# martinsbruveris/tensorflow-image-models

Measured on AMD Instinct MI355X. Metric: images/sec (fwd, bf16), higher is better.
Workload: dtype bf16; 1 GPU; resnet50 @224 fwd; per_gpu_batch=256, global_batch=256, parallelism=dp1, exchange=none, ranks=1, launcher=in-process, launch=hipGraph replay, 2 parallel branches of 128 images, branches=2

## Files before the change

### include/tfimm_hip.h

```cpp
#ifndef TFIMM_HIP_H
#define TFIMM_HIP_H

#include <stddef.h>
#include <stdint.h>

#ifdef __cplusplus
extern "C" {
#endif

#define TFIMM_HIP_ABI_VERSION 4

#if defined(__GNUC__)
#define TFIMM_API __attribute__((visibility("default")))
#else
#define TFIMM_API
#endif

#define TFIMM_EINVAL (-1)
#define TFIMM_EUNSUP (-2)

enum {
  TFIMM_ACT_NONE = 0,
  TFIMM_ACT_RELU = 1,
  TFIMM_ACT_GELU = 2,
// ... 152 lines not shown
  int64_t in_bytes;
  int64_t w_floats;
  int32_t B, c_in, H, W, c_out;
  int32_t pad_t, pad_b, pad_l, pad_r;
  int32_t taps_cap;
  int32_t lds_bytes;
} tfimm_resize_batch_aa_desc;

typedef struct tfimm_resize_batch_sizes {
  int64_t in_bytes;
  int64_t tab_elems;
  int64_t w_floats;
  int64_t n_tiles;
  int32_t max_taps;
  int32_t lds_floats;
  int32_t bad_image;
  int32_t reserved;
} tfimm_resize_batch_sizes;

TFIMM_API int tfimm_hip_resize_batch_tables(int B, const int32_t* src_hw, const int32_t* geometry, int H, int W, int c_in,
                                            const int32_t* pad, int method, int antialias, tfimm_resize_batch_sizes* sizes,
                                            tfimm_resize_batch_rec* recs, int32_t* tab_a, int32_t* tab_b, float* w);
TFIMM_API int tfimm_hip_preprocess_resize_batch(const tfimm_resize_batch_desc* d, void* stream);
TFIMM_API int tfimm_hip_preprocess_resize_batch_aa(const tfimm_resize_batch_aa_desc* d, void* stream);

typedef struct tfimm_resize_region_rec {
  int64_t in_offset;
  int64_t row_pitch;
  int32_t Hs, Ws;
  int32_t y_tab, x_tab;
  int32_t y_w, x_w;
  int32_t y_taps, x_taps;
  int32_t tile_rows;
  int32_t cols_max;
  int32_t tile0, n_tiles;
} tfimm_resize_region_rec;

typedef struct tfimm_resize_region_desc {
  const void* in;
  const tfimm_resize_region_rec* recs;
  void* out;
  const int32_t* idx;
  const float* w;
  const float* mean_host;
  const float* std_host;
  int64_t in_bytes;
  int32_t B, c_in, H, W, c_out;
  int32_t pad_t, pad_b, pad_l, pad_r;
  int32_t taps;
} tfimm_resize_region_desc;

typedef struct tfimm_resize_region_aa_desc {
  const void* in;
  const tfimm_resize_region_rec* recs;
  void* out;
  const int32_t* start;
  const int32_t* count;
  const float* w;
  const float* mean_host;
  const float* std_host;
  int64_t in_bytes;
  int64_t w_floats;
  int32_t B, c_in, H, W, c_out;
  int32_t pad_t, pad_b, pad_l, pad_r;
  int32_t taps_cap;
  int32_t lds_bytes;
} tfimm_resize_region_aa_desc;

TFIMM_API int tfimm_hip_resize_region_tables(int F, const int32_t* frame_hw, int N, const int32_t* boxes,
                                             const int32_t* box_frame, const int32_t* geometry, int H, int W, int c_in,
                                             const int32_t* pad, int method, int antialias, tfimm_resize_batch_sizes* sizes,
                                             tfimm_resize_region_rec* recs, int32_t* tab_a, int32_t* tab_b, float* w);
TFIMM_API int tfimm_hip_preprocess_regions(const tfimm_resize_region_desc* d, void* stream);
TFIMM_API int tfimm_hip_preprocess_regions_aa(const tfimm_resize_region_aa_desc* d, void* stream);

TFIMM_API int tfimm_hip_layernorm(const void* x, void* y, const float* gamma, const float* beta,
                        int64_t rows, int d, int64_t x_stride, int64_t y_stride, float eps,
                        void* stream);

typedef struct tfimm_attn_desc {
  const void* qkv;
  void* out;
  const float* rel_bias;
  int32_t batch;
  int32_t n_tokens;
  int32_t heads, hd;
  float scale;
  int32_t window, shift, res_h, res_w;
  const float* bias_log2;
} tfimm_attn_desc;

TFIMM_API int tfimm_hip_attention(const tfimm_attn_desc* d, void* stream);

typedef struct tfimm_tha_desc {
  const void* qkv;
  void* out;
  const float* proj_l_w;
  const float* proj_l_b;
  const float* proj_w_w;
  const float* proj_w_b;
  int32_t batch, n_tokens, heads, hd;
  float scale;
  const float* proj_dev;
} tfimm_tha_desc;

TFIMM_API int tfimm_hip_talking_heads_attention(const tfimm_tha_desc* d, void* stream);

TFIMM_API int tfimm_hip_class_attention(const void* q, const void* kv, void* out, int B, int n_tokens, int heads,
                              int hd, int ldq, int ldkv, int ldo, void* stream);

TFIMM_API int tfimm_hip_copy_rows(const void* src, void* dst, int B, int src_rows, int dst_rows, int dst_row0,
                        int d, void* stream);

TFIMM_API int tfimm_hip_maxpool(const void* x, void* y, int B, int H, int W, int C, int k, int stride,
                      int pad, int OH, int OW, void* stream);

TFIMM_API int tfimm_hip_mean_rows(const void* x, void* y, int B, int R, int C, int out_f32, void* stream);

TFIMM_API int tfimm_hip_bcast_rows(const void* src, void* dst, int B, int n_rows, int d,
                         int dst_rows_per_image, void* stream);

TFIMM_API int tfimm_hip_dwconv(const void* x, const float* w, const float* bias, void* y, void* sum_out,
                     int B, int H, int W, int C, int k, int stride, int pad_t, int pad_l,
                     int OH, int OW, int act, void* stream);

TFIMM_API int tfimm_hip_se_gate(const void* sums, int sums_fixed, float inv_count, const float* w1, const float* b1,
                      const float* w2, const float* b2, float* gate, int B, int C, int rd,
                      int act, int gate_act, void* stream);

TFIMM_API int tfimm_hip_scale_channels(const void* x, const float* gate, const void* residual, void* y,
                             int B, int R, int C, int act_after, void* stream);

TFIMM_API int tfimm_hip_patch_merge_ln(const void* x, void* y, const float* gamma, const float* beta,
                             int B, int H, int W, int C, float eps, void* stream);

typedef struct tfimm_chain_desc {
  const void* x;
  const void* w1;
  const float* b1;
  const void* w2;
  const float* b2;
  const void* residual;
  void* out;
  int32_t B, H, W, Cin, KH, KW, stride, pad_t, pad_l, OH, OW;
  int32_t C1, N2;
  int32_t ldw1, ldw2, ldr, ldc;
  int32_t act1, act2;
  const void* ds_x;
  const void* ds_w;
  int32_t ds_cin;
} tfimm_chain_desc;

TFIMM_API int tfimm_hip_conv_chain(const tfimm_chain_desc* d, void* stream);

typedef struct tfimm_expand_dw_desc {
  const void* x;
  const void* w1;
  const float* b1;
  const float* wdw;
  const float* b2;
  void* y;
  void* sum_out;
  int32_t B, H, W, Cin, C, Cpad, k, stride, pad_t, pad_l, OH, OW;
  int32_t act1, act2;
  int32_t stem;
  int32_t img_h, img_w;
} tfimm_expand_dw_desc;

TFIMM_API int tfimm_hip_expand_dwconv(const tfimm_expand_dw_desc* d, void* stream);

TFIMM_API int tfimm_hip_attention_probs(const void* qkv, void* probs, int B, int n_tokens, int heads, int hd,
                              float scale, void* stream);

TFIMM_API int tfimm_hip_group_norm(const void* x, const float* gamma, const float* beta, const void* residual, void* y,
                         void* stats_ws, int B, int rows, int C, int groups, float eps, int act,
                         int act_after_res, void* stream);

TFIMM_API int tfimm_hip_blur_pool(const void* x, void* y, int B, int H, int W, int C, int stride, void* stream);

TFIMM_API int tfimm_hip_avg_pool(const void* x, void* y, int B, int H, int W, int C, int k, int stride, void* stream);

TFIMM_API int tfimm_hip_eca_gate(const float* sums, float inv_count, const float* w, float* gate, int B, int C, int k,
                       int gate_act, void* stream);

TFIMM_API int tfimm_hip_grouped_conv3x3(const void* x, const void* wfrag, const float* bias, void* y, int B, int H, int W,
                              int C, int stride, int act, void* stream);

TFIMM_API int tfimm_hip_memset_async(void* dst, int value, size_t bytes, void* stream);

TFIMM_API int tfimm_hip_bias_act(const void* x, const float* bias, void* y, int64_t rows, int C, int act,
                       void* stream);

typedef struct tfimm_mlp_desc {
  const void* x;
  const void* w1;
  const float* b1;
  const void* w2;
  const float* b2;
  const void* residual;
  void* out;
  int64_t M;
  int32_t C, hidden, act;
  float eps;
} tfimm_mlp_desc;
TFIMM_API int tfimm_hip_mlp_fused(const tfimm_mlp_desc* d, void* stream);


TFIMM_API int tfimm_hip_quantize_mx(const void* x, int64_t rows, int C, int64_t x_stride, const float* gamma,
                                    const float* beta, float eps, void* q, void* q_scale, int ldq, void* stream);

typedef struct tfimm_gemm_mx_desc {
  const void* a;
  const void* a_scale;
  const void* w;
  const void* w_scale;
  const float* bias;
  const void* residual;
  void* out;
  void* out_scale;
  int32_t M, N, K;
  int32_t lda, ldw, ldr, ldc;
  int32_t out_fmt;
  int32_t act, act_after_res;
} tfimm_gemm_mx_desc;
TFIMM_API int tfimm_hip_gemm_mx(const tfimm_gemm_mx_desc* d, void* stream);


#define TFIMM_TOPK_MAX_K 64
#define TFIMM_TOPK_MAX_N 32768
TFIMM_API int tfimm_hip_topk(const float* logits, int64_t ld, int B, int N, int k, float* values, int32_t* indices,
                             float* probs, void* stream);

#define TFIMM_SCORE_MAX_N TFIMM_TOPK_MAX_N
#define TFIMM_SCORE_MAX_CONFUSION_N 4096
#define TFIMM_SCORE_IGNORE (-1)
#define TFIMM_SCORE_SCORED 0
#define TFIMM_SCORE_IGNORED 1
#define TFIMM_SCORE_INVALID 2
#define TFIMM_SCORE_LOSS_EXCLUDED 3
#define TFIMM_SCORE_LOSS_Q 4
#define TFIMM_SCORE_RANK_HIST 5
#define TFIMM_SCORE_RANK_BINS 65
#define TFIMM_SCORE_STATE_WORDS 70
TFIMM_API int tfimm_hip_score(const float* logits, int64_t ld, int B, int N, const int32_t* labels, float* loss, int32_t* rank,
                              int32_t* pred, float* prob, int64_t* state, int64_t* per_class, uint32_t* confusion, void* stream);


TFIMM_API int tfimm_hip_softmax_grad(const float* logits, int64_t ld, int B, int N, const int32_t* labels, void* grad, int64_t ldg,
                                     float* loss, int32_t* pred, void* stream);

#define TFIMM_HEAD_SGD 0
#define TFIMM_HEAD_ADAM 1
#define TFIMM_HEAD_MAX_D 8192
#define TFIMM_HEAD_MAX_C 32768
#define TFIMM_HEAD_MAX_B 65535
typedef struct tfimm_head_update_desc {
  const void* f;
  const void* g;
  const int32_t* labels;
  float* w;
  void* w16;
  float* s1;
  float* s2;
  float* bias;
  float* bias_s1;
  float* bias_s2;
  float* grad_out;
  float* bias_grad_out;
  int32_t B, D, C;
  int32_t ldf, ldg, ldw, ldw16;
  int32_t opt;
  float lr, mom_or_one_minus_b1, one_minus_b2, eps, wd2;
} tfimm_head_update_desc;
TFIMM_API int tfimm_hip_head_update(const tfimm_head_update_desc* d, void* stream);

#define TFIMM_DISTILL_MAX_E 4096
TFIMM_API int tfimm_hip_distill_grad(const float* s, int64_t ld_s, const float* t, int64_t ld_t, int B, int E, const int32_t* valid,
                                     int normalize, void* grad, int64_t ldg, float* loss, float* cosine, void* stream);


TFIMM_API int tfimm_hip_l2_normalize(const float* x, int64_t ld_x, int B, int E, float* y, int64_t ld_y, void* stream);

#define TFIMM_EMBED_MIN_E 16
#define TFIMM_EMBED_MAX_E 2048
#define TFIMM_EMBED_MAX_K 64
#define TFIMM_EMBED_MAX_B 2097120
TFIMM_API int64_t tfimm_hip_embed_search_workspace(int B, int N, int E, int k, int chunk);
TFIMM_API int tfimm_hip_embed_search(const float* q, int64_t ld_q, int B, const void* g, int64_t ld_g, int N, int E, int k, int chunk,
                                     float* scores, int32_t* indices, void* workspace, int64_t workspace_bytes, void* stream);

#define TFIMM_EMBED_WIDE_MAX_K 256
TFIMM_API int tfimm_hip_embed_search_wide_max_k(int E);
TFIMM_API int64_t tfimm_hip_embed_search_wide_workspace(int B, int N, int E, int k, int chunk);
TFIMM_API int tfimm_hip_embed_search_wide(const float* q, int64_t ld_q, int B, const void* g, int64_t ld_g, int N, int E, int k,
                                          int chunk, float* scores, int32_t* indices, void* workspace, int64_t workspace_bytes,
                                          void* stream);

#define TFIMM_EMBED_COARSE_MAX_CANDIDATES 256
TFIMM_API int tfimm_hip_embed_quantize_rows(const void* g, int64_t ld_g, int N, int E, void* codes, int64_t ld_c, int8_t* exps,
                                            void* stream);
TFIMM_API int tfimm_hip_embed_search_coarse_max_candidates(int E);
TFIMM_API int64_t tfimm_hip_embed_search_coarse_workspace(int B, int N, int E, int k, int candidates, int chunk);
TFIMM_API int tfimm_hip_embed_search_coarse(const float* q, int64_t ld_q, int B, const void* g, int64_t ld_g, const void* codes,
                                            int64_t ld_c, const int8_t* exps, int N, int E, int k, int candidates, int chunk,
                                            float* scores, int32_t* indices, void* workspace, int64_t workspace_bytes, void* stream);

// ... 95 lines not shown
```

### tensorflow-image-models_amd/csrc/gemm_chain.hip

```cpp
#include "gemm_chain_kernel.h"

#include <algorithm>
#include <cstdlib>

using namespace tfimm_gemm;

namespace {
int chain_num_cu() {
  static int n = 0;
  if (n == 0) {
    int dev = 0;
    hipDeviceProp_t prop;
    if (hipGetDevice(&dev) == hipSuccess && hipGetDeviceProperties(&prop, dev) == hipSuccess) n = prop.multiProcessorCount;
    if (n <= 0) n = 256;
  }
  return n;
}
}

int tfimm_launch_conv_strip_chain(const tfimm_chain_desc& d, int64_t M, int num_cu, hipStream_t stream);

extern "C" int tfimm_hip_conv_chain(const tfimm_chain_desc* dp, void* stream) {
  if (!dp) TFIMM_FAIL(TFIMM_EINVAL, "conv_chain: null descriptor");
  const tfimm_chain_desc& d = *dp;
  if (!d.x || !d.w1 || !d.b1 || !d.w2 || !d.b2 || !d.out) TFIMM_FAIL(TFIMM_EINVAL, "conv_chain: null pointer");
  if (d.B <= 0 || d.H <= 0 || d.W <= 0 || d.Cin <= 0 || d.KH <= 0 || d.KW <= 0 || d.stride <= 0 || d.OH <= 0 || d.OW <= 0 ||
      d.C1 <= 0 || d.N2 <= 0)
    TFIMM_FAIL(TFIMM_EINVAL, "conv_chain: bad shape");
  if (d.C1 == 128) {
    if (d.Cin != 128 || d.KH != 3 || d.KW != 3 || d.stride != 1 || d.pad_t != 1 || d.pad_l != 1 || d.OH != d.H || d.OW != d.W)
      TFIMM_FAIL(TFIMM_EUNSUP, "conv_chain: C1 = 128 is built for a 3x3 / stride 1 / pad 1 convolution over 128 -> 128 channels");
    if (d.W > 31) TFIMM_FAIL(TFIMM_EUNSUP, "conv_chain: C1 = 128 needs W <= 31 (W = %d): the strip of a 128-pixel tile must fit 192 LDS rows", d.W);
    if (d.N2 != 256 && d.N2 != 512) TFIMM_FAIL(TFIMM_EUNSUP, "conv_chain: N2 = %d (built: 256, 512)", d.N2);
    if (d.ds_x || d.ds_w) TFIMM_FAIL(TFIMM_EUNSUP, "conv_chain: the shortcut-convolution flavour exists for C1 = 64 only");
    if (d.ldw1 != 1152) TFIMM_FAIL(TFIMM_EINVAL, "conv_chain: ldw1 = %d, expected KH*KW*Cin = 1152", d.ldw1);
    if (d.ldw2 < 128 || (d.ldw2 & 7)) TFIMM_FAIL(TFIMM_EINVAL, "conv_chain: ldw2 = %d", d.ldw2);
    if (d.ldc < d.N2 || (d.ldc & 7) || (d.residual && (d.ldr < d.N2 || (d.ldr & 7))))
      TFIMM_FAIL(TFIMM_EINVAL, "conv_chain: output / residual rows must be 16-byte aligned (ldc = %d, ldr = %d)", d.ldc, d.ldr);
    if (((uintptr_t)d.x | (uintptr_t)d.w1 | (uintptr_t)d.w2 | (uintptr_t)d.out | (uintptr_t)d.residual | (uintptr_t)d.b1 | (uintptr_t)d.b2) & 15)
      TFIMM_FAIL(TFIMM_EINVAL, "conv_chain: pointers must be 16-byte aligned");
    const int64_t M = (int64_t)d.B * d.OH * d.OW;
    const int64_t big = std::max<int64_t>(M * 256, ((M - 1) * std::max(d.ldc, d.ldr) + d.N2) * 2);
    static const int64_t lim128 = getenv("TFIMM_CHAIN_LIMIT") ? std::min<int64_t>(atoll(getenv("TFIMM_CHAIN_LIMIT")), 0x7fffff00LL) : 0x7fffff00LL;
    if (big > lim128) {
      const int64_t per_img = (int64_t)d.OH * d.OW * std::max<int64_t>(256, (int64_t)std::max(d.ldc, d.ldr) * 2);
      const int64_t chunk = lim128 / per_img;
      if (chunk < 1 || d.B <= 1) TFIMM_FAIL(TFIMM_EUNSUP, "conv_chain: one image exceeds the 2 GiB a buffer descriptor addresses");
      for (int64_t b0 = 0; b0 < d.B; b0 += chunk) {
        tfimm_chain_desc c = d;
        c.B = (int32_t)std::min<int64_t>(chunk, d.B - b0);
        c.x = (const char*)d.x + b0 * d.H * d.W * 256;
        c.out = (char*)d.out + b0 * d.OH * d.OW * d.ldc * 2;
        if (d.residual) c.residual = (const char*)d.residual + b0 * d.OH * d.OW * d.ldr * 2;
        const int rc = tfimm_hip_conv_chain(&c, stream);
        if (rc != 0) return rc;
      }
      return 0;
    }
    return tfimm_launch_conv_strip_chain(d, M, chain_num_cu(), (hipStream_t)stream);
  }
  if (d.C1 != 64 || d.Cin != 64 || d.KH != 3 || d.KW != 3 || d.stride != 1 || d.pad_t != 1 || d.pad_l != 1 || d.OH != d.H ||
      d.OW != d.W)
    TFIMM_FAIL(TFIMM_EUNSUP, "conv_chain: built for a 3x3 / stride 1 / pad 1 convolution over 64 -> 64 channels");
  if (d.W > 63) TFIMM_FAIL(TFIMM_EUNSUP, "conv_chain: W = %d > 63 (the input strip of a 128-pixel tile must fit 256 LDS rows)", d.W);
  if (d.N2 != 256 && d.N2 != 512) TFIMM_FAIL(TFIMM_EUNSUP, "conv_chain: N2 = %d (built: 256, 512)", d.N2);
  const int64_t K1 = 576;
  if (d.ldw1 != K1) TFIMM_FAIL(TFIMM_EINVAL, "conv_chain: ldw1 = %d, expected KH*KW*Cin = %lld", d.ldw1, (long long)K1);
  if (d.ldw2 < d.C1 || (d.ldw2 & 7)) TFIMM_FAIL(TFIMM_EINVAL, "conv_chain: ldw2 = %d", d.ldw2);
  if (d.ldc < d.N2 || (d.ldc & 7) || (d.residual && (d.ldr < d.N2 || (d.ldr & 7))))
    TFIMM_FAIL(TFIMM_EINVAL, "conv_chain: output / residual rows must be 16-byte aligned (ldc = %d, ldr = %d)", d.ldc, d.ldr);
  if (((uintptr_t)d.x | (uintptr_t)d.w1 | (uintptr_t)d.w2 | (uintptr_t)d.out | (uintptr_t)d.residual | (uintptr_t)d.b1 |
       (uintptr_t)d.b2) & 15)
    TFIMM_FAIL(TFIMM_EINVAL, "conv_chain: pointers must be 16-byte aligned");
  const int64_t M = (int64_t)d.B * d.OH * d.OW;
  const int64_t x_bytes = (int64_t)d.B * d.H * d.W * d.Cin * 2;
  const int64_t w1_bytes = (int64_t)d.C1 * d.ldw1 * 2, w2_bytes = (int64_t)d.N2 * d.ldw2 * 2;
  const int64_t out_bytes = ((M - 1) * d.ldc + d.N2) * 2;
  const int64_t res_bytes = d.residual ? ((M - 1) * d.ldr + d.N2) * 2 : 0;
  const bool ds = d.ds_x != nullptr;
  if (ds != (d.ds_w != nullptr)) TFIMM_FAIL(TFIMM_EINVAL, "conv_chain: ds_x and ds_w go together");
  if (ds && (d.residual || d.ds_cin != 64 || (((uintptr_t)d.ds_x | (uintptr_t)d.ds_w) & 15)))
    TFIMM_FAIL(TFIMM_EUNSUP, "conv_chain: the shortcut convolution is built for a 64-channel block input and no other residual");
  if (ds && !(d.act1 == TFIMM_ACT_RELU && d.act2 == TFIMM_ACT_RELU))
    TFIMM_FAIL(TFIMM_EUNSUP, "conv_chain: the shortcut-convolution flavour is built with relu activations");
  if (w1_bytes > 0x7fffff00LL || w2_bytes > 0x7fffff00LL)
    TFIMM_FAIL(TFIMM_EUNSUP, "conv_chain: a weight tensor exceeds the 2 GiB a buffer descriptor addresses");
  static const int64_t limit = getenv("TFIMM_CHAIN_LIMIT") ? std::min<int64_t>(atoll(getenv("TFIMM_CHAIN_LIMIT")), 0x7fffff00LL) : 0x7fffff00LL;
  if (M > limit || x_bytes > limit || out_bytes > limit || res_bytes > limit) {
    const int64_t per_img = std::max<int64_t>(std::max<int64_t>((int64_t)d.H * d.W * d.Cin * 2, (int64_t)d.OH * d.OW * d.ldc * 2),
                                              d.residual ? (int64_t)d.OH * d.OW * d.ldr * 2 : 0);
    const int64_t chunk = limit / per_img;
    if (chunk < 1 || d.B <= 1) TFIMM_FAIL(TFIMM_EUNSUP, "conv_chain: one image exceeds the 2 GiB a buffer descriptor addresses");
    for (int64_t b0 = 0; b0 < d.B; b0 += chunk) {
      tfimm_chain_desc c = d;
      c.B = (int32_t)std::min<int64_t>(chunk, d.B - b0);
      c.x = (const char*)d.x + b0 * d.H * d.W * d.Cin * 2;
      c.out = (char*)d.out + b0 * d.OH * d.OW * d.ldc * 2;
      if (d.residual) c.residual = (const char*)d.residual + b0 * d.OH * d.OW * d.ldr * 2;
      if (d.ds_x) c.ds_x = (const char*)d.ds_x + b0 * d.OH * d.OW * d.ds_cin * 2;
      const int rc = tfimm_hip_conv_chain(&c, stream);
      if (rc != 0) return rc;
    }
    return 0;
  }

  ChainArgs a;
  a.x = (const bf16_t*)d.x; a.w1 = (const bf16_t*)d.w1; a.b1 = d.b1;
  a.w2 = (const bf16_t*)d.w2; a.b2 = d.b2; a.residual = (const bf16_t*)d.residual; a.out = (bf16_t*)d.out;
  a.ds_x = (const bf16_t*)d.ds_x; a.ds_w = (const uint4*)d.ds_w; a.ds_bytes = ds ? (unsigned)(M * 128) : 0u;
  a.M = (int)M; a.N2 = d.N2;
  a.B = d.B; a.H = d.H; a.W = d.W;
  a.ldw1 = d.ldw1; a.ldw2 = d.ldw2; a.ldr = d.ldr; a.ldc = d.ldc;
  a.act1 = d.act1; a.act2 = d.act2;
  a.x_bytes = (unsigned)x_bytes; a.w1_bytes = (unsigned)w1_bytes; a.w2_bytes = (unsigned)w2_bytes;
  a.out_bytes = (unsigned)out_bytes; a.res_bytes = (unsigned)res_bytes;
  a.n_tiles = (int)cdiv64(M, 128);
  {
    static const int dbg = getenv("TFIMM_CHAIN_DBG") ? atoi(getenv("TFIMM_CHAIN_DBG")) : 0;
    a.dbg = dbg;
  }

  const int vi = d.N2 == 512;
  const int ri = (d.act1 == TFIMM_ACT_RELU && d.act2 == TFIMM_ACT_RELU) ? 1 : 0;
  const gemm_chain_fn fn = ds ? (vi ? gemm_chain_kernel<8, TFIMM_ACT_RELU, true> : gemm_chain_kernel<4, TFIMM_ACT_RELU, true>)
                           : ri ? (vi ? gemm_chain_kernel<8, TFIMM_ACT_RELU> : gemm_chain_kernel<4, TFIMM_ACT_RELU>)
                                : (vi ? gemm_chain_kernel<8> : gemm_chain_kernel<4>);
  const int lds = ChainGeom::LDS_BYTES;
  static tfimm_once_t ready[2][3];
  const int fi = ds ? 2 : ri;
  if (ready[vi][fi].need()) {
    TFIMM_HIP_CHECK(hipFuncSetAttribute((const void*)fn, hipFuncAttributeMaxDynamicSharedMemorySize, lds));
    ready[vi][fi].mark();
  }
  int64_t grid = ((int64_t)chain_num_cu() * 2 + 7) / 8 * 8;
  const int64_t need = ((int64_t)a.n_tiles + 7) / 8 * 8;
  if (grid > need) grid = need;
  TFIMM_LAUNCH(fn, dim3((unsigned)grid), dim3(256), (size_t)lds, (hipStream_t)stream, a);
  return 0;
}
```

### tensorflow-image-models_amd/csrc/gemm_chain_kernel.h

```cpp
#pragma once
#include "gemm_stream_kernel.h"

namespace tfimm_gemm {

struct ChainArgs {
  const bf16_t* x;
  const bf16_t* w1;
  const float* b1;
  const bf16_t* w2;
  const float* b2;
  const bf16_t* residual;
  const bf16_t* ds_x;
  const uint4* ds_w;
  bf16_t* out;
  int M, N2;
  int B, H, W;
  int ldw1, ldw2, ldr, ldc;
  int act1, act2;
  unsigned x_bytes, w1_bytes, w2_bytes, out_bytes, res_bytes, ds_bytes;
  int n_tiles;
  int dbg;
};

typedef void (*gemm_chain_fn)(const ChainArgs);

struct ChainGeom {
  static constexpr int BM = 128, NW = 4, C1 = 64, BN2 = 64;
  static constexpr int STRIP_ROWS = 256;
  static constexpr int STRIP_BYTES = STRIP_ROWS * 128;
  static constexpr int STAGE = 64 * 128;
#ifndef TFIMM_CHAIN_NST
#define TFIMM_CHAIN_NST 2
#endif
#ifndef TFIMM_CHAIN_WTN
#define TFIMM_CHAIN_WTN 64
#endif
  static constexpr int NST = TFIMM_CHAIN_NST;
  static constexpr int WTN = TFIMM_CHAIN_WTN;
  static constexpr int EPI_WAVE = 32 * WTN * 4;
  static constexpr int LDS_BYTES = STRIP_BYTES + NST * STAGE + NW * EPI_WAVE;
  static_assert(LDS_BYTES <= 80 * 1024, "two workgroups must fit one CU's 160 KiB of LDS");
};

template <int N>
__device__ __forceinline__ void chain_wait_vm() {
  asm volatile("s_waitcnt vmcnt(%0)" ::"n"(N) : "memory");
}

template <int I>
struct ChainIdx {
  static constexpr int value = I;
};

template <int NS2, int ACT = -1, bool DS = false>
__global__ void __launch_bounds__(256, 2) gemm_chain_kernel(const ChainArgs p) {
  using G = ChainGeom;
  constexpr int BM = G::BM, NW = G::NW, STAGE = G::STAGE, BN2 = G::BN2, NST = G::NST;
  constexpr int TN1 = 2;
  constexpr int STRIP_INSTR = G::STRIP_ROWS / 8 / NW;
  constexpr int B1_INSTR = 64 / 8 / NW;
  constexpr int B2_INSTR = BN2 / 8 / NW;
  constexpr int KS2 = 4;
  constexpr int TN2 = BN2 / 32;
  constexpr int NK1 = 9;
  typedef __attribute__((ext_vector_type(4))) unsigned int u32x4;

  extern __shared__ __attribute__((aligned(16))) char smem[];
  char* const sRing = smem + G::STRIP_BYTES;
  float* const sEpi = reinterpret_cast<float*>(smem + G::STRIP_BYTES + NST * STAGE);

  const int tid = threadIdx.x;
  const int lane = tid & 63;
  const int wave = __builtin_amdgcn_readfirstlane(tid >> 6);
  const int frow = lane & 31, fhi = lane >> 5;

  int t_first, t_hi, t_step;
  {
    const int nb = gridDim.x, bid = blockIdx.x;
    const int xcd = bid & 7, j = bid >> 3;
    const int q = p.n_tiles >> 3, r = p.n_tiles & 7;
    const int t_lo = xcd * q + (xcd < r ? xcd : r);
    t_hi = t_lo + q + (xcd < r ? 1 : 0);
    t_step = nb >> 3;
    t_first = t_lo + j;
  }
  if (t_first >= t_hi) return;

  const __amdgpu_buffer_rsrc_t rsrc_x = make_rsrc(p.x, p.x_bytes);
  const __amdgpu_buffer_rsrc_t rsrc_w1 = make_rsrc(p.w1, p.w1_bytes);
  const __amdgpu_buffer_rsrc_t rsrc_w2 = make_rsrc(p.w2, p.w2_bytes);
  const __amdgpu_buffer_rsrc_t rsrc_o = make_rsrc(p.out, p.out_bytes);
  const __amdgpu_buffer_rsrc_t rsrc_r = DS ? make_rsrc(p.ds_x, p.ds_bytes) : make_rsrc(p.residual, p.res_bytes);

  static_assert(NS2 >= 2, "the counted waits below are derived for at least two GEMM-2 steps");
  constexpr int LOOK = NST - 1;
  const int lrow = lane >> 3, lpc = lane & 7;

  unsigned b1_off[B1_INSTR], b2_off[B2_INSTR];
  int strip_chunk[STRIP_INSTR];
#pragma unroll
  for (int j = 0; j < B1_INSTR; ++j) {
    const int r = (wave * B1_INSTR + j) * 8 + lrow;
    b1_off[j] = (unsigned)(((size_t)r * p.ldw1 + (lpc ^ ((r >> 1) & 7)) * 8) * 2);
  }
#pragma unroll
  for (int j = 0; j < B2_INSTR; ++j) {
    const int r = (wave * B2_INSTR + j) * 8 + lrow;
    b2_off[j] = (unsigned)(((size_t)r * p.ldw2 + (lpc ^ ((r >> 1) & 7)) * 8) * 2);
  }
#pragma unroll
  for (int j = 0; j < STRIP_INSTR; ++j) {
    const int r = (wave * STRIP_INSTR + j) * 8 + lrow;
    strip_chunk[j] = (lpc ^ ((r >> 1) & 7)) * 16;
  }
  const int halo = p.W + 1;
  const int n_pix = p.B * p.H * p.W;
  auto issue_strip = [&](int tile, bool valid) __attribute__((always_inline)) {
    const int s0 = tile * BM - halo;
#pragma unroll
    for (int j = 0; j < STRIP_INSTR; ++j) {
      const int r = (wave * STRIP_INSTR + j) * 8 + lrow;
      const int s = s0 + r;
      const bool ok = valid && s >= 0 && s < n_pix;
      const unsigned off = ok ? (unsigned)s * 128u + (unsigned)strip_chunk[j] : kOobOffset;
      __builtin_amdgcn_raw_ptr_buffer_load_lds(rsrc_x, (lds_ptr_t)(smem + (wave * STRIP_INSTR + j) * 1024), 16, (int)off, 0, 0, 0);
    }
  };
  int iss_stage = 0;
  auto issue_step = [&](auto sc, int tile) __attribute__((always_inline)) {
    constexpr int S = decltype(sc)::value;
    constexpr int SL = S >= NK1 + NS2 ? S - NK1 - NS2 : S;
    const bool valid = S >= NK1 + NS2 ? (tile + t_step < t_hi) : true;
    char* const sa = sRing + iss_stage * STAGE;
    if constexpr (SL < NK1) {
#pragma unroll
      for (int j = 0; j < B1_INSTR; ++j) {
        const unsigned off = valid ? b1_off[j] : kOobOffset;
        __builtin_amdgcn_raw_ptr_buffer_load_lds(rsrc_w1, (lds_ptr_t)(sa + (wave * B1_INSTR + j) * 1024), 16, (int)off, SL * 128, 0, 0);
      }
    } else {
      const int soff = (int)((size_t)(SL - NK1) * BN2 * p.ldw2 * 2);
#pragma unroll
      for (int j = 0; j < B2_INSTR; ++j)
        __builtin_amdgcn_raw_ptr_buffer_load_lds(rsrc_w2, (lds_ptr_t)(sa + (wave * B2_INSTR + j) * 1024), 16, (int)b2_off[j], soff, 0, 0);
    }
    iss_stage = iss_stage == NST - 1 ? 0 : iss_stage + 1;
  };

  constexpr int WTN = G::WTN, LPR = WTN / 8, RPI = 64 / LPR, ITS = 32 / RPI;
  constexpr int PASSES = BN2 / WTN;
  constexpr int BPP = WTN / 32;
  constexpr int STORES = PASSES * ITS;
  constexpr int DS_X = DS ? 4 : 0;
  constexpr int DS_W = DS ? 8 : 0;
  constexpr int EPI_LOADS = (DS ? 0 : PASSES * ITS) + PASSES * 2;
  auto epi_slot = [](int row, int slot) -> int { return WTN == 64 ? (slot ^ (row & 15)) : (slot ^ ((row >> 1) & 7)); };
  const ActParams act1p = make_act(ACT >= 0 ? ACT : p.act1), act2p = make_act(ACT >= 0 ? ACT : p.act2);
  const int e_row = lane / LPR, e_c8 = lane % LPR;
  const bool has_res = !DS && p.residual != nullptr;
  float* const sEw = sEpi + wave * (G::EPI_WAVE / 4);

  struct Ops {
    static constexpr int all(int r) {
      if (DS && r == NK1 - 2) return B1_INSTR + TN1 * 4;
      if (r < NK1 - 1) return B1_INSTR;
      if (r == NK1 - 1) return EPI_LOADS + DS_X + B1_INSTR;
      const int u = r - NK1;
      return (u < NS2 - 1 ? EPI_LOADS : 0) + DS_W + B2_INSTR + (u == 0 ? STRIP_INSTR : 0) + STORES;
    }
    static constexpr int behind_dma(int r) {
      if (r < NK1) return 0;
      return (r - NK1 == 0 ? STRIP_INSTR : 0) + STORES;
    }
    static constexpr int wait_for(int r) {
      constexpr int T = NK1 + NS2;
      int n = behind_dma((r + T - LOOK) % T);
      for (int i = 1; i < LOOK; ++i) n += all((r + T - i) % T);
      return n;
    }
  };
  static_assert(B1_INSTR == B2_INSTR, "every weight step is two pieces per wave");
  static_assert(Ops::wait_for(NK1 + NS2 - 1) < 64, "vmcnt is a 6-bit counter");

  f32x4 bias1[TN1][4];
  auto load_bias1 = [&]() __attribute__((always_inline)) {
#pragma unroll
    for (int j = 0; j < TN1; ++j)
#pragma unroll
      for (int q = 0; q < 4; ++q) {
        const float4 b4 = *reinterpret_cast<const float4*>(p.b1 + j * 32 + q * 8 + fhi * 4);
        bias1[j][q] = f32x4{b4.x, b4.y, b4.z, b4.w};
      }
  };
  if constexpr (!DS) {
    load_bias1();
    asm volatile("s_waitcnt vmcnt(0)" : "+v"(bias1[0][0]), "+v"(bias1[0][3]), "+v"(bias1[TN1 - 1][0]), "+v"(bias1[TN1 - 1][3])::"memory");
  }

  if (TFIMM_PROBE(p.dbg) & 8) {
    const int n = ((blockIdx.x >> 3) & 7) * (TFIMM_PROBE(p.dbg) >> 8);
    for (int i = 0; i < n; ++i) asm volatile("s_sleep 8");
  }
  issue_strip(t_first, true);
  issue_step(ChainIdx<0>{}, t_first);
  if constexpr (LOOK > 1) issue_step(ChainIdx<1>{}, t_first);
  if constexpr (LOOK > 2) issue_step(ChainIdx<2>{}, t_first);
  static_assert(LOOK >= 1 && LOOK <= 3, "prologue written for up to three steps of lookahead");
  int cur = 0;
  bool first = true;
  auto rotate = [&]() __attribute__((always_inline)) { cur = cur == NST - 1 ? 0 : cur + 1; };

  for (int tile = t_first; tile < t_hi; tile += t_step) {
    const int m0 = tile * BM;

    unsigned vmask;
    {
      const int m = m0 + wave * 32 + frow;
      const int hw = p.H * p.W;
      const int rem = m % hw;
      const int oy = rem / p.W, ox = rem - oy * p.W;
      const unsigned vy = (oy > 0 ? 1u : 0u) | 2u | (oy + 1 < p.H ? 4u : 0u);
      const unsigned vx = (ox > 0 ? 1u : 0u) | 2u | (ox + 1 < p.W ? 4u : 0u);
      vmask = 0;
#pragma unroll
      for (int ky = 0; ky < 3; ++ky)
        if ((vy >> ky) & 1) vmask |= vx << (3 * ky);
      if (m >= p.M) vmask = 0;
    }

    f32x16 acc1[TN1];
#pragma unroll
    for (int j = 0; j < TN1; ++j)
#pragma unroll
      for (int e = 0; e < 16; ++e) acc1[j][e] = 0.f;
    uint4 rres[2][PASSES][ITS];
    u32x4 dsx[4];
    float4 braw[2][PASSES][2];
    const int e_m = m0 + wave * 32 + e_row;
    const int em = e_m < p.M ? e_m : p.M;
    const unsigned ldc2 = (unsigned)p.ldc * 2u, ldr2 = (unsigned)p.ldr * 2u;
    auto load_epi = [&](auto uc) __attribute__((always_inline)) {
      constexpr int u = decltype(uc)::value;
      const unsigned res_off0 = (unsigned)(((size_t)em * p.ldr + u * BN2 + e_c8 * 8) * 2);
#pragma unroll
      for (int g = 0; g < PASSES; ++g) {
        if constexpr (!DS) {
#pragma unroll
        for (int it = 0; it < ITS; ++it) {
          const unsigned off = res_off0 + (unsigned)(it * RPI) * ldr2 + (unsigned)(g * WTN * 2);
          rres[u & 1][g][it] = __builtin_bit_cast(uint4, __builtin_amdgcn_raw_buffer_load_b128(rsrc_r, (int)((TFIMM_PROBE(p.dbg) & 4) ? kOobOffset : off), 0, 0));
        }
        }
        braw[u & 1][g][0] = *reinterpret_cast<const float4*>(p.b2 + u * BN2 + g * WTN + e_c8 * 8);
        braw[u & 1][g][1] = *reinterpret_cast<const float4*>(p.b2 + u * BN2 + g * WTN + e_c8 * 8 + 4);
      }
    };
    auto tap_step = [&](auto kc) __attribute__((always_inline)) {
      constexpr int k = decltype(kc)::value;
      if constexpr (k < LOOK) { if (first) chain_wait_vm<(LOOK - 1) * B1_INSTR>(); else chain_wait_vm<Ops::wait_for(k)>(); }
      else chain_wait_vm<Ops::wait_for(k)>();
      tfimm_lds_reuse_barrier();
      if constexpr (DS && k == NK1 - 2) { load_bias1(); __builtin_amdgcn_sched_barrier(0); }
      if constexpr (k == NK1 - 1) {
        load_epi(ChainIdx<0>{});
        if constexpr (DS) {
          const unsigned xo = (unsigned)(m0 + wave * 32 + frow) * 128u + (unsigned)fhi * 16u;
#pragma unroll
          for (int t = 0; t < 4; ++t) dsx[t] = __builtin_amdgcn_raw_buffer_load_b128(rsrc_r, (int)(xo + t * 32), 0, 0);
        }
        __builtin_amdgcn_sched_barrier(0);
      }
      issue_step(ChainIdx<k + LOOK>{}, tile);
      if constexpr (k == NK1 - 1) __builtin_amdgcn_sched_barrier(0);
      constexpr int ky = k / 3, kx = k % 3;
      const bool ok = (vmask >> k) & 1;
      const uint4* sB = reinterpret_cast<const uint4*>(sRing + cur * STAGE);
      const int arow = wave * 32 + frow + ky * p.W + kx;
      u32x4 ua[4];
      {
        unsigned ra[4];
#pragma unroll
        for (int ks = 0; ks < 4; ++ks) ra[ks] = (unsigned)(size_t)(lds_ptr_t)(smem + lds_slot(arow, ks * 2 + fhi) * 16);
        asm volatile("ds_read_b128 %0, %4\n\tds_read_b128 %1, %5\n\tds_read_b128 %2, %6\n\tds_read_b128 %3, %7\n\t"
                     "s_waitcnt lgkmcnt(0)"
                     : "=&v"(ua[0]), "=&v"(ua[1]), "=&v"(ua[2]), "=&v"(ua[3])
                     : "v"(ra[0]), "v"(ra[1]), "v"(ra[2]), "v"(ra[3]) : "memory");
      }
#pragma unroll
      for (int ks = 0; ks < 4; ++ks) {
        const uint4 um = sel4(ok, __builtin_bit_cast(uint4, ua[ks]));
        const bf16x8 fa = __builtin_bit_cast(bf16x8, um);
        bf16x8 fb[TN1];
#pragma unroll
        for (int j = 0; j < TN1; ++j) fb[j] = __builtin_bit_cast(bf16x8, sB[lds_slot(j * 32 + frow, ks * 2 + fhi)]);
#pragma unroll
        for (int j = 0; j < TN1; ++j)
          if (!(TFIMM_PROBE(p.dbg) & 2)) acc1[j] = __builtin_amdgcn_mfma_f32_32x32x16_bf16(fb[j], fa, acc1[j], 0, 0, 0);
      }
      rotate();
    };
    tap_step(ChainIdx<0>{}); tap_step(ChainIdx<1>{}); tap_step(ChainIdx<2>{}); tap_step(ChainIdx<3>{}); tap_step(ChainIdx<4>{});
    tap_step(ChainIdx<5>{}); tap_step(ChainIdx<6>{}); tap_step(ChainIdx<7>{}); tap_step(ChainIdx<8>{});
    bf16x8 bmid[KS2];
#pragma unroll
    for (int j = 0; j < TN1; ++j)
#pragma unroll
      for (int q2 = 0; q2 < 2; ++q2) {
        tfimm_f32x2 v[4];
#pragma unroll
        for (int h2 = 0; h2 < 2; ++h2) {
          const int q = q2 * 2 + h2;
          const f32x4 b4 = bias1[j][q];
          v[h2 * 2 + 0] = tfimm_f32x2{acc1[j][q * 4 + 0] + b4[0], acc1[j][q * 4 + 1] + b4[1]};
          v[h2 * 2 + 1] = tfimm_f32x2{acc1[j][q * 4 + 2] + b4[2], acc1[j][q * 4 + 3] + b4[3]};
        }
        act8p(v, act1p);
        bmid[j * 2 + q2] = __builtin_bit_cast(bf16x8, pack8p(v));
      }

    auto slice_step = [&](auto uc) __attribute__((always_inline)) {
      constexpr int u = decltype(uc)::value;
      constexpr int n0 = u * BN2;
      const unsigned out_off0 = (unsigned)(((size_t)em * p.ldc + n0 + e_c8 * 8) * 2);
      chain_wait_vm<Ops::wait_for(NK1 + u)>();
      tfimm_lds_reuse_barrier();
      if constexpr (u + 1 < NS2) load_epi(ChainIdx<u + 1>{});
      u32x4 wds[TN2][4];
      if constexpr (DS) {
#pragma unroll
        for (int j = 0; j < TN2; ++j)
#pragma unroll
          for (int t = 0; t < 4; ++t) wds[j][t] = __builtin_bit_cast(u32x4, p.ds_w[(size_t)((u * TN2 + j) * 4 + t) * 64 + lane]);
      }
      __builtin_amdgcn_sched_barrier(0);
      issue_step(ChainIdx<NK1 + u + LOOK>{}, tile);
      if constexpr (u == 0) issue_strip(tile + t_step, tile + t_step < t_hi);
      __builtin_amdgcn_sched_barrier(0);

      f32x16 acc[TN2];
#pragma unroll
      for (int j = 0; j < TN2; ++j)
#pragma unroll
        for (int e = 0; e < 16; ++e) acc[j][e] = 0.f;
      {
        const uint4* sW = reinterpret_cast<const uint4*>(sRing + cur * STAGE);
#pragma unroll
        for (int t = 0; t < KS2; ++t) {
          bf16x8 fw[TN2];
#pragma unroll
          for (int j = 0; j < TN2; ++j) fw[j] = __builtin_bit_cast(bf16x8, sW[lds_slot(j * 32 + frow, t * 2 + fhi)]);
#pragma unroll
          for (int j = 0; j < TN2; ++j) acc[j] = __builtin_amdgcn_mfma_f32_32x32x16_bf16(fw[j], bmid[t], acc[j], 0, 0, 0);
        }
      }
      if constexpr (DS) {
#pragma unroll
        for (int t = 0; t < 4; ++t)
#pragma unroll
          for (int j = 0; j < TN2; ++j)
            acc[j] = __builtin_amdgcn_mfma_f32_32x32x16_bf16(__builtin_bit_cast(bf16x8, wds[j][t]), __builtin_bit_cast(bf16x8, dsx[t]),
                                                             acc[j], 0, 0, 0);
      }
      rotate();

      const bool skip_epi = (TFIMM_PROBE(p.dbg) & 1) != 0;
#pragma unroll
      for (int g = 0; g < PASSES; ++g) {
        asm volatile("s_nop 15\n\ts_nop 3" : "+v"(acc[g * BPP]), "+v"(acc[g * BPP + BPP - 1]));
#pragma unroll
        for (int j = 0; j < BPP; ++j)
#pragma unroll
          for (int q = 0; q < 4; ++q) {
            const int slot = j * 8 + q * 2 + fhi;
            const f32x16& a16 = acc[g * BPP + j];
            const f32x4 v = {a16[q * 4 + 0], a16[q * 4 + 1], a16[q * 4 + 2], a16[q * 4 + 3]};
            const unsigned addr = (unsigned)(size_t)(lds_ptr_t)(&sEw[frow * WTN + epi_slot(frow, slot) * 4]);
            asm volatile("ds_write_b128 %0, %1" ::"v"(addr), "v"(v) : "memory");
          }
        const float4 bq0 = braw[u & 1][g][0], bq1 = braw[u & 1][g][1];
        const tfimm_f32x2 bias2[4] = {{bq0.x, bq0.y}, {bq0.z, bq0.w}, {bq1.x, bq1.y}, {bq1.z, bq1.w}};
#pragma unroll
        for (int ip = 0; ip < ITS; ip += 2) {
        f32x4 st[4];
        {
          unsigned ra[4];
#pragma unroll
          for (int w = 0; w < 2; ++w) {
            const int pr = (ip + w) * RPI + e_row;
            ra[2 * w] = (unsigned)(size_t)(lds_ptr_t)(&sEw[pr * WTN + epi_slot(pr, 2 * e_c8) * 4]);
            ra[2 * w + 1] = (unsigned)(size_t)(lds_ptr_t)(&sEw[pr * WTN + epi_slot(pr, 2 * e_c8 + 1) * 4]);
          }
          asm volatile("ds_read_b128 %0, %4\n\tds_read_b128 %1, %5\n\tds_read_b128 %2, %6\n\tds_read_b128 %3, %7\n\t"
                       "s_waitcnt lgkmcnt(0)"
                       : "=&v"(st[0]), "=&v"(st[1]), "=&v"(st[2]), "=&v"(st[3])
                       : "v"(ra[0]), "v"(ra[1]), "v"(ra[2]), "v"(ra[3]) : "memory");
        }
#pragma unroll
        for (int w = 0; w < 2; ++w) {
          const int it = ip + w;
          const f32x4 lo = st[2 * w], hi = st[2 * w + 1];
          tfimm_f32x2 v[4] = {{lo[0], lo[1]}, {lo[2], lo[3]}, {hi[0], hi[1]}, {hi[2], hi[3]}};
#pragma unroll
          for (int e = 0; e < 4; ++e) v[e] += bias2[e];
          if (has_res) {
            asm volatile("");
            tfimm_f32x2 r2[4];
            unpack8p(rres[u & 1][g][it], r2);
#pragma unroll
            for (int e = 0; e < 4; ++e) v[e] += r2[e];
          }
          act8p(v, act2p);
          const unsigned off = out_off0 + (unsigned)(it * RPI) * ldc2 + (unsigned)(g * WTN * 2);
          __builtin_amdgcn_raw_buffer_store_b128(__builtin_bit_cast(u32x4, pack8p(v)), rsrc_o,
                                                 (int)(skip_epi ? kOobOffset : off), 0, 0);
        }
        }
      }
    };
    slice_step(ChainIdx<0>{});
    slice_step(ChainIdx<1>{});
    if constexpr (NS2 > 2) slice_step(ChainIdx<2>{});
    if constexpr (NS2 > 3) slice_step(ChainIdx<3>{});
    if constexpr (NS2 > 4) { slice_step(ChainIdx<4>{}); slice_step(ChainIdx<5>{}); slice_step(ChainIdx<6>{}); slice_step(ChainIdx<7>{}); }
    static_assert(NS2 == 2 || NS2 == 3 || NS2 == 4 || NS2 == 8, "instantiate the slice steps of this NS2");
    first = false;
  }
  asm volatile("s_waitcnt vmcnt(0)" ::: "memory");
}

}
```

### tensorflow-image-models_amd/csrc/plan.hip

```cpp
#include "common.h"

#include <cstring>
#include <map>
#include <string>
#include <utility>
#include <vector>

namespace {

constexpr uint32_t kMagic = 0x4c504654u;
constexpr uint32_t kVersion = 1;
enum ArgKind : uint32_t { A_INT = 0, A_FLOAT = 1, A_NULL = 2, A_SLAB = 3, A_CONST = 4, A_HOST = 5, A_INPUT = 6, A_STRUCT = 7 };

struct Reader {
  const uint8_t* p;
  const uint8_t* end;
  bool ok = true;
  template <typename T> T get() {
    T v{};
    if (p + sizeof(T) > end) { ok = false; return v; }
    memcpy(&v, p, sizeof(T));
    p += sizeof(T);
    return v;
  }
  std::string str() {
    const uint32_t n = get<uint32_t>();
    if (!ok || p + n > end) { ok = false; return std::string(); }
    std::string s(reinterpret_cast<const char*>(p), n);
    p += n;
    return s;
  }
};

struct ArgSpec { uint32_t kind, aux; uint64_t value; };
struct Arg { int64_t i; double f; void* p; };
struct Reloc { uint32_t field_offset, kind, aux; uint64_t value; };
struct StructSpec { std::vector<uint8_t> bytes; std::vector<Reloc> relocs; };
struct Output { std::string name; uint32_t slab; uint64_t offset; uint64_t rows_per_image, cols; uint32_t dtype; };

typedef int (*adapter_fn)(const Arg*, void*);
struct Call { adapter_fn fn; std::string name; std::vector<ArgSpec> spec; std::vector<Arg> args; bool is_memset = false; };

template <typename T> T as(const Arg& a) {
  if constexpr (std::is_pointer<T>::value) return reinterpret_cast<T>(a.p);
  else if constexpr (std::is_floating_point<T>::value) return static_cast<T>(a.f);
  else return static_cast<T>(a.i);
}
template <typename... P, size_t... I>
int invoke_impl(int (*fn)(P..., void*), const Arg* a, void* stream, std::index_sequence<I...>) {
  return fn(as<P>(a[I])..., stream);
}
template <typename R, typename... P> constexpr size_t arity(R (*)(P...)) { return sizeof...(P) - 1; }

#define TFIMM_ADAPTER(NAME, ...)                                                                          \
  {#NAME, {[](const Arg* a, void* s) -> int {                                                             \
             return invoke_impl<__VA_ARGS__>(NAME, a, s, std::make_index_sequence<arity(NAME)>{});       \
           }, arity(NAME), 0}}
#define TFIMM_ADAPTER_DESC(NAME, DESC)                                                                    \
  {#NAME, {[](const Arg* a, void* s) -> int {                                                             \
             return invoke_impl<const DESC*>(NAME, a, s, std::make_index_sequence<arity(NAME)>{});       \
           }, arity(NAME), sizeof(DESC)}}

struct Entry { adapter_fn fn; size_t nargs; size_t desc_bytes; };

const std::map<std::string, Entry>& table() {
  using vp = const void*;
  using mp = void*;
  using fp = const float*;
  static const std::map<std::string, Entry> t = {
      TFIMM_ADAPTER_DESC(tfimm_hip_gemm, tfimm_gemm_desc),
      TFIMM_ADAPTER_DESC(tfimm_hip_conv_chain, tfimm_chain_desc),
      TFIMM_ADAPTER_DESC(tfimm_hip_mlp_fused, tfimm_mlp_desc),
      TFIMM_ADAPTER_DESC(tfimm_hip_gemm_mx, tfimm_gemm_mx_desc),
      TFIMM_ADAPTER_DESC(tfimm_hip_expand_dwconv, tfimm_expand_dw_desc),
      TFIMM_ADAPTER_DESC(tfimm_hip_stem_conv_pool, tfimm_stem_desc),
      TFIMM_ADAPTER_DESC(tfimm_hip_attention, tfimm_attn_desc),
      TFIMM_ADAPTER_DESC(tfimm_hip_talking_heads_attention, tfimm_tha_desc),
      TFIMM_ADAPTER(tfimm_hip_cast_input, vp, int, mp, int64_t, int, int),
      TFIMM_ADAPTER(tfimm_hip_cast_input_pad, vp, int, mp, int, int, int, int, int, int, int, int),
      TFIMM_ADAPTER(tfimm_hip_row_stats, vp, float*, int64_t, int, int64_t, float),
      TFIMM_ADAPTER(tfimm_hip_quantize_mx, vp, int64_t, int, int64_t, fp, fp, float, mp, mp, int),
      TFIMM_ADAPTER(tfimm_hip_layernorm, vp, mp, fp, fp, int64_t, int, int64_t, int64_t, float),
      TFIMM_ADAPTER(tfimm_hip_class_attention, vp, vp, mp, int, int, int, int, int, int, int),
      TFIMM_ADAPTER(tfimm_hip_copy_rows, vp, mp, int, int, int, int, int),
      TFIMM_ADAPTER(tfimm_hip_maxpool, vp, mp, int, int, int, int, int, int, int, int, int),
      TFIMM_ADAPTER(tfimm_hip_mean_rows, vp, mp, int, int, int, int),
      TFIMM_ADAPTER(tfimm_hip_bcast_rows, vp, mp, int, int, int, int),
      TFIMM_ADAPTER(tfimm_hip_dwconv, vp, fp, fp, mp, mp, int, int, int, int, int, int, int, int, int, int, int),
      TFIMM_ADAPTER(tfimm_hip_se_gate, vp, int, float, fp, fp, fp, fp, float*, int, int, int, int, int),
      TFIMM_ADAPTER(tfimm_hip_scale_channels, vp, fp, vp, mp, int, int, int, int),
      TFIMM_ADAPTER(tfimm_hip_patch_merge_ln, vp, mp, fp, fp, int, int, int, int, float),
      TFIMM_ADAPTER(tfimm_hip_attention_probs, vp, mp, int, int, int, int, float),
      TFIMM_ADAPTER(tfimm_hip_group_norm, vp, fp, fp, vp, mp, mp, int, int, int, int, float, int, int),
      TFIMM_ADAPTER(tfimm_hip_blur_pool, vp, mp, int, int, int, int, int),
      TFIMM_ADAPTER(tfimm_hip_avg_pool, vp, mp, int, int, int, int, int, int),
      TFIMM_ADAPTER(tfimm_hip_eca_gate, fp, float, fp, float*, int, int, int, int),
      TFIMM_ADAPTER(tfimm_hip_grouped_conv3x3, vp, vp, fp, mp, int, int, int, int, int, int),
      TFIMM_ADAPTER(tfimm_hip_bias_act, vp, fp, mp, int64_t, int, int),
      TFIMM_ADAPTER(tfimm_hip_topk, fp, int64_t, int, int, int, float*, int32_t*, float*),
  };
  return t;
}

struct Plan {
  uint32_t batch = 0;
  std::vector<uint64_t> slab_bytes, slab_off;
  std::vector<uint64_t> const_bytes, const_off, const_src;
  std::vector<std::vector<uint8_t>> host_consts;
  std::vector<StructSpec> structs;
  std::vector<Call> calls;
  std::vector<Output> outputs;
  int32_t input_call = -1;
  int32_t stem_call = -1, stem_struct = -1;
  int32_t img_h = 0, img_w = 0, img_c = 0, stem_pad_t = 0, stem_pad_l = 0;
  uint64_t workspace_bytes = 0;
  char* ws = nullptr;
};

uint64_t align256(uint64_t v) { return (v + 255) / 256 * 256; }

int parse(const void* blob, size_t bytes, Plan& pl) {
  Reader r{static_cast<const uint8_t*>(blob), static_cast<const uint8_t*>(blob) + bytes};
  if (r.get<uint32_t>() != kMagic) TFIMM_FAIL(TFIMM_EINVAL, "plan: not a plan blob");
  if (r.get<uint32_t>() != kVersion) TFIMM_FAIL(TFIMM_EINVAL, "plan: blob version mismatch");
  if ((int)r.get<uint32_t>() != tfimm_hip_abi_version()) TFIMM_FAIL(TFIMM_EINVAL, "plan: exported for another ABI version");
  pl.batch = r.get<uint32_t>();
  pl.img_h = r.get<int32_t>(); pl.img_w = r.get<int32_t>(); pl.img_c = r.get<int32_t>();
  constexpr uint64_t kMaxBuf = 1ull << 40;
  uint64_t off = 0;
  for (uint32_t i = 0, n = r.get<uint32_t>(); i < n && r.ok; ++i) {
    pl.slab_bytes.push_back(r.get<uint64_t>());
    pl.slab_off.push_back(off);
    if (pl.slab_bytes.back() > kMaxBuf || off > kMaxBuf) TFIMM_FAIL(TFIMM_EINVAL, "plan: slab %u of %llu bytes", i, (unsigned long long)pl.slab_bytes.back());
    off += align256(pl.slab_bytes.back());
  }
  for (uint32_t i = 0, n = r.get<uint32_t>(); i < n && r.ok; ++i) {
    pl.const_bytes.push_back(r.get<uint64_t>());
    pl.const_src.push_back(r.get<uint64_t>());
    pl.const_off.push_back(off);
    if (pl.const_bytes.back() > bytes || pl.const_src.back() > bytes - pl.const_bytes.back())
      TFIMM_FAIL(TFIMM_EINVAL, "plan: constant outside the blob");
    if (pl.const_bytes.back() > kMaxBuf || off > kMaxBuf) TFIMM_FAIL(TFIMM_EINVAL, "plan: workspace too large");
    off += align256(pl.const_bytes.back());
  }
  pl.workspace_bytes = off;
  for (uint32_t i = 0, n = r.get<uint32_t>(); i < n && r.ok; ++i) {
    const uint64_t nb = r.get<uint64_t>(), src = r.get<uint64_t>();
    if (nb > bytes || src > bytes - nb) TFIMM_FAIL(TFIMM_EINVAL, "plan: host constant outside the blob");
    pl.host_consts.emplace_back(static_cast<const uint8_t*>(blob) + src, static_cast<const uint8_t*>(blob) + src + nb);
  }
  for (uint32_t i = 0, n = r.get<uint32_t>(); i < n && r.ok; ++i) {
    StructSpec s;
    const uint32_t nb = r.get<uint32_t>(), nr = r.get<uint32_t>();
    if (!r.ok || nb > (size_t)(r.end - r.p)) TFIMM_FAIL(TFIMM_EINVAL, "plan: truncated struct");
    s.bytes.assign(r.p, r.p + nb);
    r.p += nb;
    for (uint32_t k = 0; k < nr && r.ok; ++k) {
      Reloc rl;
      rl.field_offset = r.get<uint32_t>(); rl.kind = r.get<uint32_t>(); rl.aux = r.get<uint32_t>(); rl.value = r.get<uint64_t>();
      if (nb < sizeof(void*) || rl.field_offset > nb - sizeof(void*)) TFIMM_FAIL(TFIMM_EINVAL, "plan: relocation outside its struct");
      s.relocs.push_back(rl);
    }
    pl.structs.push_back(std::move(s));
  }
  for (uint32_t i = 0, n = r.get<uint32_t>(); i < n && r.ok; ++i) {
    Call c;
    c.name = r.str();
    const uint32_t na = r.get<uint32_t>();
    for (uint32_t k = 0; k < na && r.ok; ++k) {
      ArgSpec a;
      a.kind = r.get<uint32_t>(); a.aux = r.get<uint32_t>(); a.value = r.get<uint64_t>();
      c.spec.push_back(a);
    }
    if (c.name == "memset") {
      c.is_memset = true;
      c.fn = nullptr;
      if (na != 2) TFIMM_FAIL(TFIMM_EINVAL, "plan: memset takes (pointer, bytes)");
    } else {
      const auto it = table().find(c.name);
      if (it == table().end()) TFIMM_FAIL(TFIMM_EUNSUP, "plan: no executor entry for %s", c.name.c_str());
      if (it->second.nargs != na) TFIMM_FAIL(TFIMM_EINVAL, "plan: %s takes %zu arguments, blob has %u", c.name.c_str(), it->second.nargs, na);
      c.fn = it->second.fn;
    }
    pl.calls.push_back(std::move(c));
  }
  pl.input_call = r.get<int32_t>();
  pl.stem_call = r.get<int32_t>(); pl.stem_struct = r.get<int32_t>();
  pl.stem_pad_t = r.get<int32_t>(); pl.stem_pad_l = r.get<int32_t>();
  for (uint32_t i = 0, n = r.get<uint32_t>(); i < n && r.ok; ++i) {
    Output o;
    o.name = r.str();
    o.slab = r.get<uint32_t>(); o.offset = r.get<uint64_t>(); o.rows_per_image = r.get<uint64_t>(); o.cols = r.get<uint64_t>();
    o.dtype = r.get<uint32_t>();
    pl.outputs.push_back(o);
  }
  if (!r.ok) TFIMM_FAIL(TFIMM_EINVAL, "plan: truncated blob");
  if (pl.input_call < 0 || pl.input_call >= (int)pl.calls.size()) TFIMM_FAIL(TFIMM_EINVAL, "plan: no input call");
  if (pl.calls[pl.input_call].spec.size() < 2) TFIMM_FAIL(TFIMM_EINVAL, "plan: the input call takes (pointer, dtype, ...)");
  if (pl.stem_call >= 0) {
    if (pl.stem_call >= (int)pl.calls.size() || pl.stem_struct < 0 || pl.stem_struct >= (int)pl.structs.size() ||
        pl.structs[pl.stem_struct].bytes.size() < sizeof(tfimm_stem_desc))
      TFIMM_FAIL(TFIMM_EINVAL, "plan: bad stem reference");
  }
  for (const auto& o : pl.outputs) {
    if (o.slab >= pl.slab_off.size()) TFIMM_FAIL(TFIMM_EINVAL, "plan: output '%s' outside its slab", o.name.c_str());
    if (o.dtype > 2) TFIMM_FAIL(TFIMM_EINVAL, "plan: output '%s' has dtype code %u (0 bf16, 1 fp32, 2 int32)", o.name.c_str(), o.dtype);
    const uint64_t cap = pl.slab_bytes[o.slab], esz = o.dtype == 0 ? 2 : 4;
    bool ok = o.offset < cap && o.cols > 0 && o.rows_per_image > 0 && pl.batch > 0 && o.cols <= kMaxBuf && o.rows_per_image <= kMaxBuf / pl.batch;
    if (ok) {
      const uint64_t rows = o.rows_per_image * (uint64_t)pl.batch;
      ok = o.cols <= kMaxBuf / rows && rows * o.cols <= (cap - o.offset) / esz;
    }
    if (!ok) TFIMM_FAIL(TFIMM_EINVAL, "plan: output '%s' outside its slab", o.name.c_str());
  }
  for (const auto& c : pl.calls) {
    if (c.is_memset) continue;
    const auto& e = table().find(c.name)->second;
    for (size_t k = 0; k < c.spec.size(); ++k)
      if (c.spec[k].kind == A_STRUCT) {
        if (c.spec[k].aux >= pl.structs.size()) TFIMM_FAIL(TFIMM_EINVAL, "plan: bad struct reference");
        if (e.desc_bytes && pl.structs[c.spec[k].aux].bytes.size() < e.desc_bytes)
          TFIMM_FAIL(TFIMM_EINVAL, "plan: %s descriptor has %zu bytes, the entry point reads %zu", c.name.c_str(),
                     pl.structs[c.spec[k].aux].bytes.size(), e.desc_bytes);
      }
// ... 132 lines not shown
```

### tensorflow-image-models_amd/tfimm/engine/ffi.py

```python
import ctypes as C
import os

import torch

_HERE = os.path.dirname(os.path.abspath(__file__))
LIB_PATH = os.environ.get("TFIMM_HIP_LIB") or os.path.join(_HERE, "libtfimm_hip.so")

ACT = {
    "": 0, "linear": 0, "none": 0, None: 0,
    "relu": 1, "gelu": 2, "swish": 3, "sigmoid": 4, "relu6": 5, "tanh": 6,
}
A_DENSE, A_CONV, A_CONV_C4 = 0, 1, 2


class GemmDesc(C.Structure):
    _fields_ = [
        ("a", C.c_void_p), ("wt", C.c_void_p), ("bias", C.c_void_p), ("residual", C.c_void_p),
        ("out", C.c_void_p), ("a_scale", C.c_void_p),
        ("M", C.c_int32), ("N", C.c_int32), ("K", C.c_int32),
        ("lda", C.c_int32), ("ldw", C.c_int32), ("ldr", C.c_int32), ("ldc", C.c_int32),
        ("out_f32", C.c_int32), ("act", C.c_int32), ("act_after_res", C.c_int32),
        ("res_mod", C.c_int32),
        ("remap_in", C.c_int32), ("remap_out", C.c_int32), ("remap_off", C.c_int32),
        ("mode", C.c_int32),
        ("B", C.c_int32), ("H", C.c_int32), ("W", C.c_int32), ("Cin", C.c_int32),
        ("KH", C.c_int32), ("KW", C.c_int32), ("stride", C.c_int32),
        ("pad_t", C.c_int32), ("pad_l", C.c_int32), ("OH", C.c_int32), ("OW", C.c_int32),
        ("rows_per_image", C.c_int32), ("tile_hint", C.c_int32), ("stride_w", C.c_int32),
        ("pix_pitch", C.c_int32),
        ("ln_stats", C.c_void_p), ("ln_c1", C.c_void_p),
        ("a2", C.c_void_p), ("K2", C.c_int32), ("lda2", C.c_int32),
        ("a2_stride", C.c_int32), ("a2_H", C.c_int32), ("a2_W", C.c_int32), ("a2_OH", C.c_int32), ("a2_OW", C.c_int32),
        ("a2_window", C.c_int32),
    ]


class AttnDesc(C.Structure):
    _fields_ = [
        ("qkv", C.c_void_p), ("out", C.c_void_p), ("rel_bias", C.c_void_p),
        ("batch", C.c_int32), ("n_tokens", C.c_int32), ("heads", C.c_int32), ("hd", C.c_int32),
        ("scale", C.c_float),
        ("window", C.c_int32), ("shift", C.c_int32), ("res_h", C.c_int32), ("res_w", C.c_int32),
        ("bias_log2", C.c_void_p),
    ]


class ThaDesc(C.Structure):
    _fields_ = [
        ("qkv", C.c_void_p), ("out", C.c_void_p),
        ("proj_l_w", C.c_void_p), ("proj_l_b", C.c_void_p), ("proj_w_w", C.c_void_p), ("proj_w_b", C.c_void_p),
        ("batch", C.c_int32), ("n_tokens", C.c_int32), ("heads", C.c_int32), ("hd", C.c_int32),
        ("scale", C.c_float), ("proj_dev", C.c_void_p),
    ]


class StemDesc(C.Structure):
    _fields_ = [
        ("x", C.c_void_p), ("wt", C.c_void_p), ("bias", C.c_void_p), ("out", C.c_void_p),
        ("batch", C.c_int32), ("Hp", C.c_int32), ("Wp2", C.c_int32), ("OH", C.c_int32), ("OW", C.c_int32),
        ("ldw", C.c_int32),
        ("in_dtype", C.c_int32), ("H", C.c_int32), ("W", C.c_int32), ("pad_t", C.c_int32), ("pad_l", C.c_int32),
    ]


class ChainDesc(C.Structure):
    _fields_ = [
        ("x", C.c_void_p), ("w1", C.c_void_p), ("b1", C.c_void_p), ("w2", C.c_void_p), ("b2", C.c_void_p),
        ("residual", C.c_void_p), ("out", C.c_void_p),
        ("B", C.c_int32), ("H", C.c_int32), ("W", C.c_int32), ("Cin", C.c_int32), ("KH", C.c_int32), ("KW", C.c_int32),
        ("stride", C.c_int32), ("pad_t", C.c_int32), ("pad_l", C.c_int32), ("OH", C.c_int32), ("OW", C.c_int32),
        ("C1", C.c_int32), ("N2", C.c_int32),
        ("ldw1", C.c_int32), ("ldw2", C.c_int32), ("ldr", C.c_int32), ("ldc", C.c_int32),
        ("act1", C.c_int32), ("act2", C.c_int32),
        ("ds_x", C.c_void_p), ("ds_w", C.c_void_p), ("ds_cin", C.c_int32),
    ]


class ExpandDwDesc(C.Structure):
    _fields_ = [
        ("x", C.c_void_p), ("w1", C.c_void_p), ("b1", C.c_void_p), ("wdw", C.c_void_p), ("b2", C.c_void_p),
        ("y", C.c_void_p), ("sum_out", C.c_void_p),
        ("B", C.c_int32), ("H", C.c_int32), ("W", C.c_int32), ("Cin", C.c_int32), ("C", C.c_int32), ("Cpad", C.c_int32),
        ("k", C.c_int32), ("stride", C.c_int32), ("pad_t", C.c_int32), ("pad_l", C.c_int32), ("OH", C.c_int32),
        ("OW", C.c_int32), ("act1", C.c_int32), ("act2", C.c_int32),
        ("stem", C.c_int32), ("img_h", C.c_int32), ("img_w", C.c_int32),
    ]


class MlpDesc(C.Structure):
    _fields_ = [("x", C.c_void_p), ("w1", C.c_void_p), ("b1", C.c_void_p), ("w2", C.c_void_p),
                ("b2", C.c_void_p), ("residual", C.c_void_p), ("out", C.c_void_p), ("M", C.c_int64),
                ("C", C.c_int32), ("hidden", C.c_int32), ("act", C.c_int32), ("eps", C.c_float)]


class GemmMxDesc(C.Structure):
    _fields_ = [("a", C.c_void_p), ("a_scale", C.c_void_p), ("w", C.c_void_p), ("w_scale", C.c_void_p),
                ("bias", C.c_void_p), ("residual", C.c_void_p), ("out", C.c_void_p), ("out_scale", C.c_void_p),
                ("M", C.c_int32), ("N", C.c_int32), ("K", C.c_int32),
                ("lda", C.c_int32), ("ldw", C.c_int32), ("ldr", C.c_int32), ("ldc", C.c_int32),
                ("out_fmt", C.c_int32), ("act", C.c_int32), ("act_after_res", C.c_int32)]


class LoraDesc(C.Structure):
    _fields_ = [("x", C.c_void_p), ("a", C.c_void_p), ("b", C.c_void_p), ("residual", C.c_void_p), ("out", C.c_void_p),
                ("M", C.c_int64), ("K", C.c_int32), ("N", C.c_int32), ("Rp", C.c_int32),
                ("lda", C.c_int32), ("lda_a", C.c_int32), ("ldr", C.c_int32), ("ldc", C.c_int32)]


class HeadUpdateDesc(C.Structure):
    _fields_ = [("f", C.c_void_p), ("g", C.c_void_p), ("labels", C.c_void_p),
                ("w", C.c_void_p), ("w16", C.c_void_p), ("s1", C.c_void_p), ("s2", C.c_void_p),
                ("bias", C.c_void_p), ("bias_s1", C.c_void_p), ("bias_s2", C.c_void_p),
                ("grad_out", C.c_void_p), ("bias_grad_out", C.c_void_p),
                ("B", C.c_int32), ("D", C.c_int32), ("C", C.c_int32),
                ("ldf", C.c_int32), ("ldg", C.c_int32), ("ldw", C.c_int32), ("ldw16", C.c_int32),
                ("opt", C.c_int32),
                ("lr", C.c_float), ("mom_or_one_minus_b1", C.c_float), ("one_minus_b2", C.c_float), ("eps", C.c_float),
                ("wd2", C.c_float)]


class ResizeDesc(C.Structure):
    _fields_ = [("in_", C.c_void_p), ("out", C.c_void_p),
                ("y_idx", C.c_void_p), ("y_w", C.c_void_p), ("x_idx", C.c_void_p), ("x_w", C.c_void_p),
                ("mean_host", C.POINTER(C.c_float)), ("std_host", C.POINTER(C.c_float)),
                ("B", C.c_int32), ("Hs", C.c_int32), ("Ws", C.c_int32), ("c_in", C.c_int32),
                ("H", C.c_int32), ("W", C.c_int32), ("c_out", C.c_int32),
                ("pad_t", C.c_int32), ("pad_b", C.c_int32), ("pad_l", C.c_int32), ("pad_r", C.c_int32),
                ("taps", C.c_int32)]


class ResizeAADesc(C.Structure):
    _fields_ = [("in_", C.c_void_p), ("out", C.c_void_p),
                ("y_start", C.c_void_p), ("y_count", C.c_void_p), ("y_w", C.c_void_p),
                ("x_start", C.c_void_p), ("x_count", C.c_void_p), ("x_w", C.c_void_p),
                ("mean_host", C.POINTER(C.c_float)), ("std_host", C.POINTER(C.c_float)),
                ("B", C.c_int32), ("Hs", C.c_int32), ("Ws", C.c_int32), ("c_in", C.c_int32),
                ("H", C.c_int32), ("W", C.c_int32), ("c_out", C.c_int32),
                ("pad_t", C.c_int32), ("pad_b", C.c_int32), ("pad_l", C.c_int32), ("pad_r", C.c_int32),
                ("y_taps", C.c_int32), ("x_taps", C.c_int32)]


class ResizeBatchRec(C.Structure):
    _fields_ = [("in_offset", C.c_int64), ("Hs", C.c_int32), ("Ws", C.c_int32),
                ("y_tab", C.c_int32), ("x_tab", C.c_int32), ("y_w", C.c_int32), ("x_w", C.c_int32),
                ("y_taps", C.c_int32), ("x_taps", C.c_int32),
                ("tile_rows", C.c_int32), ("cols_max", C.c_int32), ("tile0", C.c_int32), ("n_tiles", C.c_int32)]


class ResizeBatchDesc(C.Structure):
    _fields_ = [("in_", C.c_void_p), ("recs", C.c_void_p), ("out", C.c_void_p),
                ("idx", C.c_void_p), ("w", C.c_void_p),
                ("mean_host", C.POINTER(C.c_float)), ("std_host", C.POINTER(C.c_float)),
                ("in_bytes", C.c_int64),
                ("B", C.c_int32), ("c_in", C.c_int32), ("H", C.c_int32), ("W", C.c_int32), ("c_out", C.c_int32),
                ("pad_t", C.c_int32), ("pad_b", C.c_int32), ("pad_l", C.c_int32), ("pad_r", C.c_int32),
                ("taps", C.c_int32)]


class ResizeBatchAADesc(C.Structure):
    _fields_ = [("in_", C.c_void_p), ("recs", C.c_void_p), ("out", C.c_void_p),
                ("start", C.c_void_p), ("count", C.c_void_p), ("w", C.c_void_p),
                ("mean_host", C.POINTER(C.c_float)), ("std_host", C.POINTER(C.c_float)),
                ("in_bytes", C.c_int64), ("w_floats", C.c_int64),
                ("B", C.c_int32), ("c_in", C.c_int32), ("H", C.c_int32), ("W", C.c_int32), ("c_out", C.c_int32),
                ("pad_t", C.c_int32), ("pad_b", C.c_int32), ("pad_l", C.c_int32), ("pad_r", C.c_int32),
                ("taps_cap", C.c_int32), ("lds_bytes", C.c_int32)]


class ResizeRegionRec(C.Structure):
    _fields_ = [("in_offset", C.c_int64), ("row_pitch", C.c_int64)] + ResizeBatchRec._fields_[1:]


class ResizeRegionDesc(C.Structure):
    _fields_ = ResizeBatchDesc._fields_


class ResizeRegionAADesc(C.Structure):
    _fields_ = ResizeBatchAADesc._fields_


class ResizeBatchSizes(C.Structure):
    _fields_ = [("in_bytes", C.c_int64), ("tab_elems", C.c_int64), ("w_floats", C.c_int64), ("n_tiles", C.c_int64),
                ("max_taps", C.c_int32), ("lds_floats", C.c_int32), ("bad_image", C.c_int32), ("reserved", C.c_int32)]


_vp, _i, _i64, _f = C.c_void_p, C.c_int, C.c_int64, C.c_float
SYMBOLS = {
    "tfimm_hip_abi_version": (_i, []),
    "tfimm_hip_last_error": (C.c_char_p, []),
    "tfimm_hip_device_info": (_i, [_i, C.c_char_p, _i]),
    "tfimm_hip_gemm": (_i, [C.POINTER(GemmDesc), _vp]),
    "tfimm_hip_conv_chain": (_i, [C.POINTER(ChainDesc), _vp]),
    "tfimm_hip_mlp_fused": (_i, [C.POINTER(MlpDesc), _vp]),
    "tfimm_hip_gemm_mx": (_i, [C.POINTER(GemmMxDesc), _vp]),
    "tfimm_hip_quantize_mx": (_i, [_vp, _i64, _i, _i64, _vp, _vp, _f, _vp, _vp, _i, _vp]),
    "tfimm_hip_expand_dwconv": (_i, [C.POINTER(ExpandDwDesc), _vp]),
    "tfimm_hip_stem_conv_pool": (_i, [C.POINTER(StemDesc), _vp]),
    "tfimm_hip_cast_input": (_i, [_vp, _i, _vp, _i64, _i, _i, _vp]),
    "tfimm_hip_cast_input_pad": (_i, [_vp, _i, _vp, _i, _i, _i, _i, _i, _i, _i, _i, _vp]),
    "tfimm_hip_preprocess_input": (_i, [_vp, _vp, _i64, _i, _i, C.POINTER(C.c_float), C.POINTER(C.c_float), _vp]),
    "tfimm_hip_preprocess_input_pad": (_i, [_vp, _vp, _i, _i, _i, _i, _i, _i, _i, _i, C.POINTER(C.c_float),
                                            C.POINTER(C.c_float), _vp]),
    "tfimm_hip_resize_taps": (_i, [_i, _i, _i, _i, _i, C.POINTER(C.c_int32), C.POINTER(C.c_float)]),
    "tfimm_hip_preprocess_resize": (_i, [C.POINTER(ResizeDesc), _vp]),
    "tfimm_hip_resize_span_taps": (_i, [_i, _i, _i]),
    "tfimm_hip_resize_spans": (_i, [_i, _i, _i, _i, _i, C.POINTER(C.c_int32), C.POINTER(C.c_int32), C.POINTER(C.c_float)]),
    "tfimm_hip_preprocess_resize_aa": (_i, [C.POINTER(ResizeAADesc), _vp]),
    "tfimm_hip_resize_batch_tables": (_i, [_i, C.POINTER(C.c_int32), C.POINTER(C.c_int32), _i, _i, _i, C.POINTER(C.c_int32), _i, _i,
                                           C.POINTER(ResizeBatchSizes), _vp, _vp, _vp, _vp]),
    "tfimm_hip_preprocess_resize_batch": (_i, [C.POINTER(ResizeBatchDesc), _vp]),
    "tfimm_hip_preprocess_resize_batch_aa": (_i, [C.POINTER(ResizeBatchAADesc), _vp]),
    "tfimm_hip_resize_region_tables": (_i, [_i, C.POINTER(C.c_int32), _i, C.POINTER(C.c_int32), C.POINTER(C.c_int32),
                                            C.POINTER(C.c_int32), _i, _i, _i, C.POINTER(C.c_int32), _i, _i,
                                            C.POINTER(ResizeBatchSizes), _vp, _vp, _vp, _vp]),
    "tfimm_hip_preprocess_regions": (_i, [C.POINTER(ResizeRegionDesc), _vp]),
    "tfimm_hip_preprocess_regions_aa": (_i, [C.POINTER(ResizeRegionAADesc), _vp]),
    "tfimm_hip_row_stats": (_i, [_vp, _vp, _i64, _i, _i64, _f, _vp]),
    "tfimm_hip_layernorm": (_i, [_vp, _vp, _vp, _vp, _i64, _i, _i64, _i64, _f, _vp]),
    "tfimm_hip_attention": (_i, [C.POINTER(AttnDesc), _vp]),
    "tfimm_hip_talking_heads_attention": (_i, [C.POINTER(ThaDesc), _vp]),
    "tfimm_hip_class_attention": (_i, [_vp, _vp, _vp, _i, _i, _i, _i, _i, _i, _i, _vp]),
    "tfimm_hip_copy_rows": (_i, [_vp, _vp, _i, _i, _i, _i, _i, _vp]),
    "tfimm_hip_maxpool": (_i, [_vp, _vp, _i, _i, _i, _i, _i, _i, _i, _i, _i, _vp]),
    "tfimm_hip_mean_rows": (_i, [_vp, _vp, _i, _i, _i, _i, _vp]),
    "tfimm_hip_bcast_rows": (_i, [_vp, _vp, _i, _i, _i, _i, _vp]),
    "tfimm_hip_dwconv": (_i, [_vp, _vp, _vp, _vp, _vp, _i, _i, _i, _i, _i, _i, _i, _i, _i, _i, _i, _vp]),
    "tfimm_hip_se_gate": (_i, [_vp, _i, _f, _vp, _vp, _vp, _vp, _vp, _i, _i, _i, _i, _i, _vp]),
    "tfimm_hip_scale_channels": (_i, [_vp, _vp, _vp, _vp, _i, _i, _i, _i, _vp]),
    "tfimm_hip_patch_merge_ln": (_i, [_vp, _vp, _vp, _vp, _i, _i, _i, _i, _f, _vp]),
    "tfimm_hip_attention_probs": (_i, [_vp, _vp, _i, _i, _i, _i, _f, _vp]),
    "tfimm_hip_group_norm": (_i, [_vp, _vp, _vp, _vp, _vp, _vp, _i, _i, _i, _i, _f, _i, _i, _vp]),
    "tfimm_hip_blur_pool": (_i, [_vp, _vp, _i, _i, _i, _i, _i, _vp]),
    "tfimm_hip_avg_pool": (_i, [_vp, _vp, _i, _i, _i, _i, _i, _i, _vp]),
    "tfimm_hip_eca_gate": (_i, [_vp, _f, _vp, _vp, _i, _i, _i, _i, _vp]),
    "tfimm_hip_grouped_conv3x3": (_i, [_vp, _vp, _vp, _vp, _i, _i, _i, _i, _i, _i, _vp]),
    "tfimm_hip_bias_act": (_i, [_vp, _vp, _vp, _i64, _i, _i, _vp]),
    "tfimm_hip_topk": (_i, [_vp, _i64, _i, _i, _i, _vp, _vp, _vp, _vp]),
    "tfimm_hip_score": (_i, [_vp, _i64, _i, _i, _vp, _vp, _vp, _vp, _vp, _vp, _vp, _vp, _vp]),
    "tfimm_hip_softmax_grad": (_i, [_vp, _i64, _i, _i, _vp, _vp, _i64, _vp, _vp, _vp]),
    "tfimm_hip_head_update": (_i, [C.POINTER(HeadUpdateDesc), _vp]),
    "tfimm_hip_distill_grad": (_i, [_vp, _i64, _vp, _i64, _i, _i, _vp, _i, _vp, _i64, _vp, _vp, _vp]),
    "tfimm_hip_l2_normalize": (_i, [_vp, _i64, _i, _i, _vp, _i64, _vp]),
    "tfimm_hip_embed_search_workspace": (_i64, [_i, _i, _i, _i, _i]),
    "tfimm_hip_embed_search": (_i, [_vp, _i64, _i, _vp, _i64, _i, _i, _i, _i, _vp, _vp, _vp, _i64, _vp]),
    "tfimm_hip_embed_search_wide_max_k": (_i, [_i]),
    "tfimm_hip_embed_search_wide_workspace": (_i64, [_i, _i, _i, _i, _i]),
    "tfimm_hip_embed_search_wide": (_i, [_vp, _i64, _i, _vp, _i64, _i, _i, _i, _i, _vp, _vp, _vp, _i64, _vp]),
    "tfimm_hip_embed_quantize_rows": (_i, [_vp, _i64, _i, _i, _vp, _i64, _vp, _vp]),
    "tfimm_hip_embed_search_coarse_max_candidates": (_i, [_i]),
    "tfimm_hip_embed_search_coarse_workspace": (_i64, [_i, _i, _i, _i, _i, _i]),
    "tfimm_hip_embed_search_coarse": (_i, [_vp, _i64, _i, _vp, _i64, _vp, _i64, _vp, _i, _i, _i, _i, _i, _vp, _vp, _vp, _i64, _vp]),
    "tfimm_hip_knn_vote": (_i, [_vp, _vp, _i64, _i, _i, _vp, _i, _vp, _f, _i, _i, _vp, _vp, _vp, _vp, _vp]),
    "tfimm_hip_knn_score": (_i, [_vp, _vp, _i64, _i, _i, _vp, _i, _vp, _f, _i, _vp, _vp, _vp, _vp, _vp, _vp, _vp, _vp, _vp]),
    "tfimm_hip_cluster_assign": (_i, [_vp, _i64, _i, _vp, _i64, _i, _i, _vp, _vp, _vp]),
    "tfimm_hip_segment_mean_workspace": (_i64, [_i, _i, _i]),
    "tfimm_hip_segment_mean": (_i, [_vp, _i64, _i, _i, _vp, _i, _vp, _i, _vp, _i64, _vp, _vp, _i64, _vp]),
    "tfimm_hip_lora_delta": (_i, [C.POINTER(LoraDesc), _vp]),
    "tfimm_hip_plan_query": (_i, [_vp, C.c_size_t, _vp]),
    "tfimm_hip_plan_create": (_i, [_vp, C.c_size_t, _vp, _vp, C.POINTER(_vp)]),
    "tfimm_hip_plan_forward": (_i, [_vp, _vp, _i, _vp]),
    "tfimm_hip_plan_output": (_i, [_vp, C.c_char_p, C.POINTER(_vp), C.POINTER(_i64), C.POINTER(_i64), C.POINTER(_i)]),
    "tfimm_hip_plan_destroy": (_i, [_vp]),
    "tfimm_hip_ref_gemm": (_i, [C.POINTER(GemmDesc), _vp]),
    "tfimm_hip_ref_cast_input": (_i, [_vp, _i, _vp, _i64, _i, _i, C.POINTER(C.c_float), C.POINTER(C.c_float), _vp]),
    "tfimm_hip_ref_preprocess_resize": (_i, [C.POINTER(ResizeDesc), _vp]),
    "tfimm_hip_ref_preprocess_resize_aa": (_i, [C.POINTER(ResizeAADesc), _vp]),
    "tfimm_hip_ref_preprocess_resize_batch": (_i, [C.POINTER(ResizeBatchDesc), _vp]),
    "tfimm_hip_ref_preprocess_resize_batch_aa": (_i, [C.POINTER(ResizeBatchAADesc), _vp]),
    "tfimm_hip_ref_preprocess_regions": (_i, [C.POINTER(ResizeRegionDesc), _vp]),
    "tfimm_hip_ref_preprocess_regions_aa": (_i, [C.POINTER(ResizeRegionAADesc), _vp]),
    "tfimm_hip_ref_layernorm": (_i, [_vp, _vp, _vp, _vp, _i64, _i, _i64, _i64, _f, _vp]),
    "tfimm_hip_ref_patch_merge_ln": (_i, [_vp, _vp, _vp, _vp, _i, _i, _i, _i, _f, _vp]),
    "tfimm_hip_ref_copy_rows": (_i, [_vp, _vp, _i, _i, _i, _i, _i, _vp]),
    "tfimm_hip_ref_bcast_rows": (_i, [_vp, _vp, _i, _i, _i, _i, _vp]),
    "tfimm_hip_ref_mean_rows": (_i, [_vp, _vp, _i, _i, _i, _i, _vp]),
    "tfimm_hip_ref_scale_channels": (_i, [_vp, _vp, _vp, _vp, _i, _i, _i, _i, _vp]),
    "tfimm_hip_ref_maxpool": (_i, [_vp, _vp, _i, _i, _i, _i, _i, _i, _i, _i, _i, _vp]),
    "tfimm_hip_ref_avg_pool": (_i, [_vp, _vp, _i, _i, _i, _i, _i, _i, _vp]),
    "tfimm_hip_ref_blur_pool": (_i, [_vp, _vp, _i, _i, _i, _i, _i, _vp]),
    "tfimm_hip_ref_dwconv": (_i, [_vp, _vp, _vp, _vp, _vp, _i, _i, _i, _i, _i, _i, _i, _i, _i, _i, _i, _vp]),
    "tfimm_hip_ref_group_norm": (_i, [_vp, _vp, _vp, _vp, _vp, _vp, _i, _i, _i, _i, _f, _i, _i, _vp]),
    "tfimm_hip_ref_attention": (_i, [C.POINTER(AttnDesc), _vp]),
    "tfimm_hip_ref_attention_probs": (_i, [_vp, _vp, _i, _i, _i, _i, _f, _vp]),
    "tfimm_hip_ref_talking_heads_attention": (_i, [C.POINTER(ThaDesc), _vp]),
    "tfimm_hip_ref_class_attention": (_i, [_vp, _vp, _vp, _i, _i, _i, _i, _i, _i, _i, _vp]),
    "tfimm_hip_ref_lora_delta": (_i, [C.POINTER(LoraDesc), _vp]),
    "tfimm_hip_memset_async": (_i, [_vp, _i, C.c_size_t, _vp]),
}


class PlanInfo(C.Structure):
    _fields_ = [("workspace_bytes", C.c_uint64), ("batch", C.c_int32), ("in_h", C.c_int32), ("in_w", C.c_int32),
                ("in_c", C.c_int32), ("n_calls", C.c_int32), ("n_outputs", C.c_int32)]


class HipError(RuntimeError):
    pass


def _load():
    if not os.path.exists(LIB_PATH):
        raise ImportError(
            f"{LIB_PATH} not found: build it with `make -C tensorflow-image-models_amd/csrc -j8` "
            "(or __graft_entry__.build()). tfimm has no CPU fallback."
        )
    lib = C.CDLL(LIB_PATH)
    for name, (res, args) in SYMBOLS.items():
        fn = getattr(lib, name)
        fn.restype = res
        fn.argtypes = args
    v = lib.tfimm_hip_abi_version()
    if v != 4 and not (v == 3 and os.environ.get("TFIMM_HIP_LIB")):
        raise ImportError("libtfimm_hip.so ABI version mismatch")
    return lib


lib = _load()
ABI = lib.tfimm_hip_abi_version()


_dp_lib = None


def dp_lib():
    global _dp_lib
    if _dp_lib is None:
        path = os.environ.get("TFIMM_HIP_DP_LIB") or os.path.join(_HERE, "libtfimm_hip_dp.so")
        if not os.path.exists(path):
            raise HipError(f"{path} not found: build it with `make -C tensorflow-image-models_amd/csrc`")
        L = C.CDLL(path)
        L.tfimm_hip_dp_abi_version.restype = C.c_int
        L.tfimm_hip_dp_last_error.restype = C.c_char_p
        L.tfimm_hip_dp_shard_bounds.argtypes = [C.c_int64, C.c_int, C.c_int, C.POINTER(C.c_int64), C.POINTER(C.c_int64)]
        L.tfimm_hip_dp_unique_id.argtypes = [C.c_void_p, C.c_size_t]
        L.tfimm_hip_dp_create.argtypes = [C.POINTER(C.c_void_p), C.c_void_p, C.c_size_t, C.c_int, C.c_int, C.c_int]
        L.tfimm_hip_dp_world.argtypes = [C.c_void_p, C.POINTER(C.c_int), C.POINTER(C.c_int)]
        L.tfimm_hip_dp_all_gather_logits.argtypes = [C.c_void_p, C.c_void_p, C.c_void_p, C.c_int64, C.c_int64, C.c_void_p]
        L.tfimm_hip_dp_forward.argtypes = [C.c_void_p, C.c_void_p, C.c_void_p, C.c_int, C.c_void_p, C.c_int64, C.c_void_p, C.c_void_p]
        L.tfimm_hip_dp_destroy.argtypes = [C.c_void_p]
        for f in ("shard_bounds", "unique_id", "create", "world", "all_gather_logits", "forward", "destroy"):
            getattr(L, "tfimm_hip_dp_" + f).restype = C.c_int
        assert L.tfimm_hip_dp_abi_version() == 1
        _dp_lib = L
    return _dp_lib

# ... 221 lines not shown
```

### tensorflow-image-models_amd/tfimm/engine/graph.py

```python
import ctypes as C
import os
import zlib
from dataclasses import dataclass, field
from typing import Callable, Dict, List, Optional, Tuple

import numpy as np

from ..utils.etc import same_padding
from . import pack, precision, tune


@dataclass
class TRef:
    id: int
    rows: int
    C: int
    H: int = 0
    W: int = 0
    dtype: str = "bf16"
    keep: bool = False
    name: str = ""

    @property
    def itemsize(self) -> int:
        return {"bf16": 2, "f32": 4, "i32": 4, "mx": 1}[self.dtype]

    @property
    def mx_ld(self) -> int:
        return pack.ceil_to(self.C, pack.MX_KPAD)

    @property
    def bytes_per_image(self) -> int:
        if self.dtype == "mx":
            return self.rows * (self.mx_ld + self.mx_ld // pack.MX_BLOCK)
        return self.rows * self.C * self.itemsize


@dataclass
class Const:
    id: int
    host: Optional[np.ndarray]
    name: str = ""
    nbytes: int = 0
    keep_host: bool = False
    key: Optional[tuple] = None


@dataclass
class Op:
    kind: str
    inputs: List[int]
    output: Optional[int]
    consts: Dict[str, int]
    attrs: Dict[str, object]
    cite: str = ""
    extra_outputs: List[int] = field(default_factory=list)


class Program:
    def __init__(self):
        self.precision = precision.get()
        self.tensors: List[TRef] = []
        self.consts: List[Const] = []
        self.ops: List[Op] = []
        self.input: Optional[TRef] = None
        self.input_shape: Tuple[int, int, int] = (0, 0, 0)
        self.outputs: Dict[str, TRef] = {}
        self._dev_consts = None
        self._dev_consts_device = None
        self.const_cache: Optional[dict] = None

    def new_tensor(self, rows, C, H=0, W=0, dtype="bf16", name="") -> TRef:
        if dtype == "bf16" and self.precision == "fp32":
            dtype = "f32"
        t = TRef(len(self.tensors), int(rows), int(C), int(H), int(W), dtype, False, name)
        self.tensors.append(t)
        return t

    def new_const(self, host: np.ndarray, name="", keep_host=False) -> int:
        h = np.ascontiguousarray(host)
        key = (name, h.shape, h.dtype.str, zlib.crc32(h.view(np.uint8).reshape(-1)))
        c = Const(len(self.consts), h, name, h.nbytes, keep_host, key)
        self.consts.append(c)
        return c.id

    def add(self, kind, inputs, output, consts=None, cite="", extra_outputs=(), **attrs) -> Op:
        op = Op(kind, [t.id for t in inputs], None if output is None else output.id,
                consts or {}, attrs, cite, [t.id for t in extra_outputs])
        self.ops.append(op)
        return op

    def mark_output(self, name: str, t: TRef):
        self.tensors[t.id].keep = True
        self.outputs[name] = t

    def flops_per_image(self) -> int:
        total = 0
        for op in self.ops:
            a = op.attrs
            if op.kind in ("gemm", "gemm_mx", "stem_pool"):
                total += 2 * a["M"] * a["N"] * a["K_true"]
            elif op.kind in ("attention", "talking_heads_attention", "conv_chain", "mlp_fused"):
                total += a["flops"]
            elif op.kind == "dwconv":
                total += 2 * a["OH"] * a["OW"] * a["C"] * a["k"] * a["k"]
            elif op.kind in ("grouped_conv", "expand_dwconv"):
                total += a["flops"]
        return total

    def weight_bytes(self) -> int:
        return sum(c.nbytes for c in self.consts)

    def plan_buffers(self) -> Tuple[Dict[int, int], List[int]]:
        last_use: Dict[int, int] = {}
        for i, op in enumerate(self.ops):
            for t in op.inputs:
                last_use[t] = i
            for t in ([op.output] if op.output is not None else []) + op.extra_outputs:
                last_use[t] = max(last_use.get(t, i), i)
        slabs: List[int] = []
        free: List[int] = []
        assign: Dict[int, int] = {}
        for i, op in enumerate(self.ops):
            outs = ([op.output] if op.output is not None else []) + op.extra_outputs
            for out in outs:
                if out in assign:
                    continue
                need = self.tensors[out].bytes_per_image
                best = None
                for s_ in free:
                    if slabs[s_] >= need and (best is None or slabs[s_] < slabs[best]):
                        best = s_
                if best is None and free:
                    best = max(free, key=lambda s_: slabs[s_])
                    slabs[best] = need
                if best is None:
                    slabs.append(need)
                    best = len(slabs) - 1
                else:
                    free.remove(best)
                assign[out] = best
            for t in set(op.inputs + outs):
                if last_use.get(t) == i and not self.tensors[t].keep and t in assign:
                    if assign[t] not in free:
                        free.append(assign[t])
        return assign, slabs

    def upload(self, device="cuda"):
        import torch
        if self._dev_consts is not None and self._dev_consts_device == device:
            return
        self._dev_consts_device = device
        cache = self.const_cache if self.const_cache is not None else {}
        dev = []
        for c in self.consts:
            ck = (device,) + c.key
            t = cache.get(ck)
            if t is None:
                h = c.host
                if h is None:
                    src = next((v for k, v in cache.items() if k[1:] == c.key), None)
                    if src is None:
                        raise RuntimeError(f"constant {c.key!r}: no host copy and no uploaded copy to take it from")
                    t = src.to(device)
                elif h.dtype == np.uint16:
                    t = torch.from_numpy(h.view(np.int16).copy()).to(device)
                else:
                    t = torch.from_numpy(h.copy()).to(device)
                cache[ck] = t
            dev.append(t)
            if not c.keep_host and device != "cpu":
                c.host = None
        self._dev_consts = dev

    def make_plan(self, batch: int, device: str = "cuda") -> "Plan":
        return Plan(self, batch, device)

    def fuse_mx_outputs(self) -> int:
        readers: Dict[int, List[int]] = {}
        for i, op in enumerate(self.ops):
            for t in op.inputs:
                readers.setdefault(t, []).append(i)
        drop = set()
        for op in self.ops:
            if op.kind != "gemm_mx" or op.attrs["out_fmt"] != 0:
                continue
            t = self.tensors[op.output]
            r = readers.get(t.id, [])
            if t.keep or len(r) != 1:
                continue
            q = self.ops[r[0]]
            if q.kind != "quant_mx" or q.attrs["ln"] or t.C % pack.MX_KPAD:
                continue
            op.output = q.output
            op.attrs["out_fmt"] = 2
            drop.add(r[0])
        self.ops = [op for i, op in enumerate(self.ops) if i not in drop]
        return len(drop)

    def live_across(self, op_index: int) -> List[int]:
        written, needed = set(), set()
        for i, op in enumerate(self.ops):
            outs = ([op.output] if op.output is not None else []) + list(op.extra_outputs)
            if i < op_index:
                written.update(outs)
            else:
                needed.update(op.inputs)
                needed.update(o for o in outs if o in written)
        keep = {t.id for t in self.tensors if t.keep}
        return sorted(t for t in written if t in needed or t in keep)

    def supports_branches(self) -> bool:
        return True

    def make_branches(self, batch: int, parts: int = 2, device: str = "cuda") -> List["Plan"]:
        return [Plan(self, nb, device) for nb in branch_sizes(batch, parts)]


def branch_sizes(batch: int, parts: int) -> List[int]:
    parts = max(1, min(int(parts), int(batch)))
    return [batch // parts + (1 if i < batch % parts else 0) for i in range(parts)]


class Builder:
    def __init__(self, weights: Dict[str, np.ndarray]):
        self.w = weights
        self._orig_w = weights
        self.p = Program()
        self.fp32 = self.p.precision == "fp32"
        self.fp8 = self.p.precision == "fp8"

    def finish(self) -> Program:
        if self.fp8:
            self.p.fuse_mx_outputs()
        return self.p

    def wget(self, name: str) -> np.ndarray:
        if name not in self.w:
            raise KeyError(f"missing weight '{name}'")
        return np.asarray(self.w[name], dtype=np.float32)

    def define(self, name: str, value: np.ndarray) -> str:
        if self.w is self._orig_w:
            self.w = dict(self._orig_w)
        self.w[name] = np.asarray(value, dtype=np.float32)
        return name

    def act_const(self, value: np.ndarray, name: str) -> int:
        v = np.ascontiguousarray(value, dtype=np.float32)
        return self.p.new_const(v if self.fp32 else pack.to_bf16_bits(v), name)

    def bn(self, prefix: str, eps: float):
        return pack.bn_scale_shift(self.wget(prefix + "/gamma"), self.wget(prefix + "/beta"),
                                   self.wget(prefix + "/moving_mean"),
                                   self.wget(prefix + "/moving_variance"), eps)

    def image_input(self, H: int, W: int, cin: int) -> TRef:
        p = self.p
        cpad = cin if self.fp32 else pack.pad_channels(cin)
        raw = p.new_tensor(H * W, cin, H, W, dtype="raw", name="input")
        raw.keep = True
        p.input = raw
        p.input_shape = (H, W, cin)
        x = p.new_tensor(H * W, cpad, H, W, name="input_bf16")
        self._cast_op = p.add("cast_input", [raw], x, c_in=cin, c_out=cpad, H=H, W=W, pad=(0, 0, 0, 0),
                              cite="Keras input autocast")
        self._cast_out = x.id
        return x

    def conv(self, x: TRef, kernel: str, *, stride=1, padding=0, bn: Optional[str] = None,
             bn_eps=1e-5, bias: Optional[str] = None, act="", residual: Optional[TRef] = None,
             act_after_res=False, a_scale: Optional[TRef] = None, flatten=False,
             remap=None, res_const=None, res_mod=0, then_maxpool=None, flops_k: Optional[int] = None,
             fold_shortcut=None, cite="", name="") -> TRef:
        p = self.p
        k = self.wget(kernel)
        kh, kw, cin, cout = k.shape
# ... 596 lines not shown

        def padc(a):
            out = np.zeros(a.shape[:-1] + (cpad,), np.float32)
            out[..., :c] = a
            return out
        consts = {"w1": p.new_const(w1, stem_kernel + ":frag"), "b1": p.new_const(padc(np.asarray(t1, np.float32)), stem_kernel + ":bias"),
                  "wdw": p.new_const(padc(wd), dw_kernel + ":pad"), "b2": p.new_const(padc(b2), dw_kernel + ":bias")}
        out = p.new_tensor(OH * OW, c, OH, OW, name=dw_kernel)
        sums = p.new_tensor(1, 2 * c, dtype="f32", name=dw_kernel + ":sums") if squeeze else None
        p.add("expand_dwconv", [x], out, consts, cite=cite, extra_outputs=[sums] if sums is not None else [],
              H=SH, W=SW, Cin=4, C=c, Cpad=cpad, k=3, stride=1, pad_t=dpt, pad_l=dpl, OH=OH, OW=OW, act=act,
              sums=None if sums is None else sums.id, stem=1, img_h=hp, img_w=wp,
              flops=2 * SH * SW * 9 * cin * c + 2 * OH * OW * c * 9)
        return out, sums

    def se_gate(self, sums: TRef, count: int, w_reduce: str, b_reduce: str, w_expand: str, b_expand: str,
                act: str, gate_act="sigmoid", cite="") -> TRef:
        p = self.p
        w1 = self.wget(w_reduce)
        w2 = self.wget(w_expand)
        c, rd = w1.shape[2], w1.shape[3]
        consts = {
            "w1": p.new_const(np.ascontiguousarray(w1[0, 0].T), w_reduce),
            "b1": p.new_const(self.wget(b_reduce), b_reduce),
            "w2": p.new_const(np.ascontiguousarray(w2[0, 0]), w_expand),
            "b2": p.new_const(self.wget(b_expand), b_expand),
        }
        gate = p.new_tensor(1, c, dtype="f32", name="se_gate")
        fixed = sums.C == 2 * c
        assert fixed or sums.C == c
        if getattr(sums, "is_mean", False):
            count = 1
        p.add("se_gate", [sums], gate, consts, cite=cite, C=c, rd=rd, inv_count=1.0 / count, act=act,
              gate_act=gate_act, sums_fixed=1 if fixed else 0)
        return gate

    def scale_channels(self, x: TRef, gate: TRef, residual: Optional[TRef] = None, relu_after=False, cite="") -> TRef:
        out = self.p.new_tensor(x.rows, x.C, x.H, x.W, name="se_scaled")
        ins = [x, gate] + ([residual] if residual is not None else [])
        self.p.add("scale_channels", ins, out, cite=cite, R=x.rows, C=x.C, has_residual=residual is not None,
                   act_after=1 if relu_after else 0)
        return out

    def group_norm(self, x: TRef, prefix: str, groups: int, eps: float, *, act="", residual: Optional[TRef] = None,
                   act_after="", cite="") -> TRef:
        p = self.p
        g, b = self.wget(prefix + "/gamma"), self.wget(prefix + "/beta")
        assert g.shape[0] == x.C and x.C % groups == 0, f"{prefix}: {x.C} channels, {groups} groups"
        out = p.new_tensor(x.rows, x.C, x.H, x.W, name=prefix)
        ws = p.new_tensor(1, 4 * groups, dtype="f32", name=prefix + ":stats")
        consts = {"gamma": p.new_const(g, prefix + "/gamma"), "beta": p.new_const(b, prefix + "/beta")}
        ins = [x] + ([residual] if residual is not None else [])
        if residual is not None:
            assert residual.rows == x.rows and residual.C == x.C
        p.add("group_norm", ins, out, consts, cite=cite, extra_outputs=[ws], rows=x.rows, C=x.C, groups=groups,
              eps=float(eps), act=act, act_after=act_after, has_residual=residual is not None, ws=ws.id)
        return out

    def blur_pool(self, x: TRef, stride: int, cite="") -> TRef:
        pad = (3 + stride) // 2 - 1
        OH, OW = (x.H + 2 * pad - 3) // stride + 1, (x.W + 2 * pad - 3) // stride + 1
        out = self.p.new_tensor(OH * OW, x.C, OH, OW, name="blur_pool")
        self.p.add("blur_pool", [x], out, cite=cite, H=x.H, W=x.W, C=x.C, stride=stride)
        return out

    def avg_pool(self, x: TRef, k: int, stride: int, cite="") -> TRef:
        OH, OW = -(-x.H // stride), -(-x.W // stride)
        out = self.p.new_tensor(OH * OW, x.C, OH, OW, name="avg_pool")
        self.p.add("avg_pool", [x], out, cite=cite, H=x.H, W=x.W, C=x.C, k=k, stride=stride)
        return out

    def eca_gate(self, mean: TRef, kernel: str, gate_act="sigmoid", cite="") -> TRef:
        assert mean.dtype == "f32" and mean.rows == 1
        w = np.ascontiguousarray(self.wget(kernel).reshape(-1), dtype=np.float32)
        gate = self.p.new_tensor(1, mean.C, dtype="f32", name="eca_gate")
        self.p.add("eca_gate", [mean], gate, {"w": self.p.new_const(w, kernel)}, cite=cite, C=mean.C, k=int(w.shape[0]),
                   gate_act=gate_act)
        return gate

    def patch_merge_ln(self, x: TRef, prefix: str, eps: float, cite="") -> TRef:
        p = self.p
        g, b = self.wget(prefix + "/gamma"), self.wget(prefix + "/beta")
        assert g.shape[0] == 4 * x.C
        out = p.new_tensor((x.H // 2) * (x.W // 2), 4 * x.C, x.H // 2, x.W // 2, name="patch_merge")
        consts = {"gamma": p.new_const(g, prefix + "/gamma"), "beta": p.new_const(b, prefix + "/beta")}
        p.add("patch_merge_ln", [x], out, consts, cite=cite, H=x.H, W=x.W, C=x.C, eps=float(eps))
        return out

    def topk(self, logits: TRef, k: int, probs=True, heads: int = 1, cite="tf.nn.softmax + tf.math.top_k behind model(x)"):
        from . import ffi
        p = self.p
        k, heads = int(k), int(heads)
        if logits.dtype != "f32":
            raise ValueError(f"topk reads float32 logits, got a {logits.dtype} tensor (a model without classifier has none)")
        assert heads >= 1 and logits.C % heads == 0, (logits.C, heads)
        N = logits.C // heads
        if N > ffi.TOPK_MAX_N:
            raise ValueError(f"topk: {N} classes, more than TFIMM_TOPK_MAX_N = {ffi.TOPK_MAX_N} (the row is held in LDS)")
        if not 1 <= k <= min(N, ffi.TOPK_MAX_K):
            raise ValueError(f"topk: k={k}, must be in [1, min({N} classes, TFIMM_TOPK_MAX_K = {ffi.TOPK_MAX_K})]")
        rows = logits.rows * heads
        values = p.new_tensor(rows, k, dtype="f32", name="topk_values")
        indices = p.new_tensor(rows, k, dtype="i32", name="topk_indices")
        pr = p.new_tensor(rows, k, dtype="f32", name="topk_probs") if probs else None
        p.add("topk", [logits], values, cite=cite, extra_outputs=[indices] + ([pr] if probs else []),
              rows=rows, N=N, k=k, ld=logits.C // heads, probs=bool(probs))
        p.mark_output("topk_values", values)
        p.mark_output("topk_indices", indices)
        if probs:
            p.mark_output("topk_probs", pr)
        return values, indices, pr

    def l2_normalize(self, x: TRef, cite="tf.math.l2_normalize(x, axis=-1)", name="") -> TRef:
        if x.dtype != "f32":
            raise ValueError(f"l2_normalize reads a float32 tensor, got {x.dtype}")
        out = self.p.new_tensor(x.rows, x.C, x.H, x.W, dtype="f32", name=name or "l2_normalize")
        self.p.add("l2_normalize", [x], out, cite=cite, rows=x.rows, E=x.C)
        return out

    def reshape(self, x: TRef, rows: int, C: int, H=0, W=0) -> TRef:
        assert rows * C == x.rows * x.C
        out = TRef(x.id, rows, C, H, W, x.dtype, x.keep, x.name)
        return out


class _Mixed:
    dtype = "torch.uint8"

    def __repr__(self):
        return "MIXED"


MIXED = _Mixed()


class _Regions:
    dtype = "torch.uint8"

    def __repr__(self):
        return "REGIONS"


REGIONS = _Regions()


def _grown(need: int, have: int, floor: int) -> int:
    cap = max(have, floor)
    while cap < need:
        cap *= 2
    return cap


class Plan:
    def __init__(self, prog: Program, batch: int, device: str = "cuda", external: Optional[Dict[int, int]] = None):
        import torch
        from . import ffi
        self.ffi = ffi
        self.external = dict(external or {})
        self.op_call_start: List[int] = []
        self.prog = prog
        self.batch = batch
        self.device = device
        prog.upload(device)
        assign, slabs = prog.plan_buffers()
        self.slab_bytes = [s * batch for s in slabs]
        self.slabs = [torch.empty(max(n, 16), dtype=torch.uint8, device=device) for n in self.slab_bytes]
        self.assign = assign
        self._keepalive = []
        self.calls: List[Tuple[Callable, tuple]] = []
        self._input_patch = None
        self._input_call = None
        self._input_pad = (0, 0, 0, 0)
        self._stem_raw = None
        self._resize_tabs: Dict[tuple, tuple] = {}
        self._mixed: Dict[tuple, dict] = {}
        self._regions: Dict[tuple, dict] = {}
        self._gemm_descs = []
        self._gemm_call_index = []
        self._tune_times = {}
        self._build()
        if prog.precision == "fp32":
            self._bind_fp32()
        elif device != "cpu" and tune.autotune_enabled():
            self.autotune()

    def tptr(self, tid: int) -> int:
        if tid in self.external:
            return self.external[tid]
        return self.slabs[self.assign[tid]].data_ptr()

    def mx_ptrs(self, t: TRef) -> Tuple[int, int]:
        base = self.tptr(t.id)
        return base, base + self.batch * t.rows * t.mx_ld

    def cptr(self, cid: Optional[int]) -> Optional[int]:
        if cid is None:
            return None
        return self.prog._dev_consts[cid].data_ptr()

    def tensor_view(self, t: TRef):
        import torch
        slab = self.slabs[self.assign[t.id]]
        n = self.batch * t.rows * t.C
        if t.dtype == "f32":
            return slab[: n * 4].view(torch.float32).view(self.batch, t.rows, t.C)
        if t.dtype == "i32":
            return slab[: n * 4].view(torch.int32).view(self.batch, t.rows, t.C)
        return slab[: n * 2].view(torch.bfloat16).view(self.batch, t.rows, t.C)

    def _build(self):
        ffi, lib, B = self.ffi, self.ffi.lib, self.batch
        prog = self.prog
        for op in prog.ops:
            a = op.attrs
            k = op.kind
            self.op_call_start.append(len(self.calls))
            if k == "cast_input":
                out = self.tptr(op.output)
                H, W, cin = prog.input_shape
                self._input_patch = (len(self.calls), out, B * H * W, a["c_in"], a["c_out"])
                self._input_pad = tuple(a["pad"])
                if a["pad"] != (0, 0, 0, 0):
                    pt_, pb_, pl_, pr_ = a["pad"]
                    self._input_call = (lib.tfimm_hip_cast_input_pad, (out, B, H, W, a["c_in"], pt_, pb_, pl_, pr_))
                    self._input_call_u8 = (lib.tfimm_hip_preprocess_input_pad, self._input_call[1])
                else:
                    self._input_call = (lib.tfimm_hip_cast_input, (out, B * H * W, a["c_in"], a["c_out"]))
                    self._input_call_u8 = (lib.tfimm_hip_preprocess_input, self._input_call[1])
                self.calls.append((self._input_call[0], None))
            elif k == "gemm":
                d = ffi.GemmDesc()
                a_ptr = self.tptr(op.inputs[0])
                d.mode = a["mode"]
                d.M = a["M"] * B
                d.N, d.K = a["N"], a["K"]
                d.ldw = a["ldw"]
                if a["mode"] == 0:
                    d.lda = a["lda"]
                    a_ptr += a.get("a_byte_offset", 0)
                    d.rows_per_image = a.get("a_rows_per_image", 0)
                else:
                    d.B, d.H, d.W, d.Cin = B, a["H"], a["W"], a["Cin"]
                    d.KH, d.KW, d.stride = a["KH"], a["KW"], a["stride"]
                    d.pad_t, d.pad_l, d.OH, d.OW = a["pad_t"], a["pad_l"], a["OH"], a["OW"]
                    d.stride_w = a.get("stride_w", 0)
                    d.pix_pitch = a.get("pix_pitch", 0)
                    a_ptr += a.get("a_byte_offset", 0)
                d.a = a_ptr
                d.wt = self.cptr(op.consts["wt"])
                d.bias = self.cptr(op.consts.get("bias"))
                out_t = prog.tensors[op.output]
                out_ptr = self.tptr(out_t.id) + a.get("out_col", 0) * out_t.itemsize + a.get("out_byte_offset", 0)
                d.out = out_ptr
                d.ldc = a.get("ldc", out_t.C)
                d.out_f32 = a["out_f32"]
                d.act = ffi.ACT[a["act"]]
                d.act_after_res = 1 if a["act_after_res"] else 0
                idx = 1
                if a.get("ln"):
                    d.ln_stats = self.tptr(op.inputs[idx])
                    d.ln_c1 = self.cptr(op.consts["ln_c1"])
                    idx += 1
                if a.get("has_residual"):
                    d.residual = self.tptr(op.inputs[idx]) + a.get("res_byte_offset", 0)
                    idx += 1
                    d.ldr = a["ldr"]
                elif "residual" in op.consts:
                    d.residual = self.cptr(op.consts["residual"])
                    d.ldr = a["N"]
                d.res_mod = a.get("res_mod", 0)
                if a.get("has_scale"):
                    d.a_scale = self.tptr(op.inputs[idx])
                    d.rows_per_image = a["a_rows_per_image"]
                if a.get("remap"):
                    d.remap_in, d.remap_out, d.remap_off = a["remap"]
                if a.get("dual"):
                    du = a["dual"]
                    d.a2 = self.tptr(op.inputs[idx])
                    idx += 1
                    d.K2, d.lda2, d.a2_stride = du["K2"], du["lda2"], du["stride"]
                    d.a2_H, d.a2_W, d.a2_OH, d.a2_OW = du["H"], du["W"], du["OH"], du["OW"]
                    d.a2_window = du.get("window", 0)
                d.tile_hint = tune.lookup(d)
                self._keepalive.append(d)
                self._gemm_descs.append(d)
                self._gemm_call_index.append(len(self.calls))
                self.calls.append((lib.tfimm_hip_gemm, (C.byref(d),)))
            elif k == "quant_mx":
                x_t, q_t = prog.tensors[op.inputs[0]], prog.tensors[op.output]
                q, qs = self.mx_ptrs(q_t)
                self.calls.append((lib.tfimm_hip_quantize_mx,
                                   (self.tptr(x_t.id), B * a["rows"], a["C"], x_t.C, self.cptr(op.consts.get("gamma")),
                                    self.cptr(op.consts.get("beta")), a["eps"], q, qs, q_t.mx_ld)))
            elif k == "gemm_mx":
                d = ffi.GemmMxDesc()
                a_t, out_t = prog.tensors[op.inputs[0]], prog.tensors[op.output]
                d.a, d.a_scale = self.mx_ptrs(a_t)
                d.w, d.w_scale = self.cptr(op.consts["w"]), self.cptr(op.consts["w_scale"])
                d.bias = self.cptr(op.consts.get("bias"))
                if a["out_fmt"] == 2:
                    d.out, d.out_scale = self.mx_ptrs(out_t)
                else:
                    d.out = self.tptr(out_t.id)
                d.M, d.N, d.K = a["M"] * B, a["N"], a["K"]
                d.lda, d.ldw, d.ldc = a_t.mx_ld, pack.ceil_to(a["K"], pack.MX_KPAD), out_t.C
                d.out_fmt = a["out_fmt"]
                d.act, d.act_after_res = ffi.ACT[a["act"]], 0
                if a["has_residual"]:
                    d.residual = self.tptr(op.inputs[1])
                    d.ldr = prog.tensors[op.inputs[1]].C
                self._keepalive.append(d)
                self.calls.append((lib.tfimm_hip_gemm_mx, (C.byref(d),)))
            elif k == "conv_chain":
                d = ffi.ChainDesc()
                d.x = self.tptr(op.inputs[0])
                d.w1, d.b1 = self.cptr(op.consts["w1"]), self.cptr(op.consts["b1"])
                d.w2, d.b2 = self.cptr(op.consts["w2"]), self.cptr(op.consts["b2"])
                d.residual = self.tptr(op.inputs[1]) if a["has_residual"] else None
                if a.get("has_ds"):
                    d.ds_x, d.ds_w, d.ds_cin = self.tptr(op.inputs[-1]), self.cptr(op.consts["ds_w"]), 64
                d.out = self.tptr(op.output)
                d.B, d.H, d.W, d.Cin, d.KH, d.KW = B, a["H"], a["W"], a["Cin"], a["KH"], a["KW"]
                d.stride, d.pad_t, d.pad_l, d.OH, d.OW = a["stride"], a["pad"], a["pad"], a["OH"], a["OW"]
                d.C1, d.N2, d.ldw1, d.ldw2, d.ldr, d.ldc = a["C1"], a["N2"], a["ldw1"], a["ldw2"], a["N2"], a["N2"]
                d.act1, d.act2 = ffi.ACT[a["act1"]], ffi.ACT[a["act2"]]
                self._keepalive.append(d)
                self.calls.append((lib.tfimm_hip_conv_chain, (C.byref(d),)))
            elif k == "mlp_fused":
                d = ffi.MlpDesc()
                d.x, d.residual, d.out = self.tptr(op.inputs[0]), self.tptr(op.inputs[1]), self.tptr(op.output)
                d.w1, d.b1 = self.cptr(op.consts["w1"]), self.cptr(op.consts["b1"])
                d.w2, d.b2 = self.cptr(op.consts["w2"]), self.cptr(op.consts["b2"])
                d.M, d.C, d.hidden, d.act, d.eps = B * a["rows"], a["C"], a["hidden"], ffi.ACT[a["act"]], a["eps"]
                self._keepalive.append(d)
                self.calls.append((lib.tfimm_hip_mlp_fused, (C.byref(d),)))
            elif k == "expand_dwconv":
                d = ffi.ExpandDwDesc()
                d.x, d.y = self.tptr(op.inputs[0]), self.tptr(op.output)
                d.w1, d.b1 = self.cptr(op.consts["w1"]), self.cptr(op.consts["b1"])
                d.wdw, d.b2 = self.cptr(op.consts["wdw"]), self.cptr(op.consts["b2"])
                d.sum_out = None
                if a["sums"] is not None:
                    d.sum_out = self.tptr(a["sums"])
                    self.calls.append(("memset", (d.sum_out, B * a["C"] * 8)))
                d.B, d.H, d.W, d.Cin, d.C, d.Cpad = B, a["H"], a["W"], a["Cin"], a["C"], a["Cpad"]
                d.k, d.stride, d.pad_t, d.pad_l, d.OH, d.OW = a["k"], a["stride"], a["pad_t"], a["pad_l"], a["OH"], a["OW"]
                d.act1 = d.act2 = ffi.ACT[a["act"]]
                d.stem, d.img_h, d.img_w = a.get("stem", 0), a.get("img_h", 0), a.get("img_w", 0)
                self._keepalive.append(d)
                self.calls.append((lib.tfimm_hip_expand_dwconv, (C.byref(d),)))
            elif k == "grouped_conv":
                self.calls.append((lib.tfimm_hip_grouped_conv3x3,
                                   (self.tptr(op.inputs[0]), self.cptr(op.consts["w"]), self.cptr(op.consts["bias"]),
                                    self.tptr(op.output), B, a["H"], a["W"], a["C"], a["stride"], ffi.ACT[a["act"]])))
            elif k == "row_stats":
                self.calls.append((lib.tfimm_hip_row_stats,
                                   (self.tptr(op.inputs[0]), self.tptr(op.output), B * a["rows"], a["d"], a["d"], a["eps"])))
            elif k == "layernorm":
                xp = self.tptr(op.inputs[0]) + a["x_byte_offset"]
                self.calls.append((lib.tfimm_hip_layernorm,
                                   (xp, self.tptr(op.output) + a["y_byte_offset"], self.cptr(op.consts["gamma"]),
                                    self.cptr(op.consts["beta"]), B * a["rows"], a["d"], a["x_stride"],
                                    a["y_stride"], a["eps"])))
            elif k == "attention":
                d = ffi.AttnDesc()
                d.qkv = self.tptr(op.inputs[0])
                d.out = self.tptr(op.output)
                d.rel_bias = self.cptr(op.consts.get("rel_bias"))
                d.bias_log2 = self.cptr(op.consts.get("bias_log2"))
                d.batch, d.n_tokens, d.heads, d.hd = B, a["n_tokens"], a["heads"], a["hd"]
                d.scale = a["scale"]
                d.window, d.shift, d.res_h, d.res_w = a["window"], a["shift"], a["res_h"], a["res_w"]
                self._keepalive.append(d)
                self.calls.append((lib.tfimm_hip_attention, (C.byref(d),)))
            elif k == "talking_heads_attention":
                d = ffi.ThaDesc()
                d.qkv = self.tptr(op.inputs[0])
                d.out = self.tptr(op.output)
                host = {r: prog.consts[op.consts[r]].host for r in ("wl", "bl", "ww", "bw")}
                self._keepalive.append(host)
                d.proj_l_w, d.proj_l_b = host["wl"].ctypes.data, host["bl"].ctypes.data
                d.proj_w_w, d.proj_w_b = host["ww"].ctypes.data, host["bw"].ctypes.data
                d.proj_dev = self.cptr(op.consts["dev"])
                d.batch, d.n_tokens, d.heads, d.hd, d.scale = B, a["n_tokens"], a["heads"], a["hd"], a["scale"]
                self._keepalive.append(d)
                self.calls.append((lib.tfimm_hip_talking_heads_attention, (C.byref(d),)))
            elif k == "class_attention":
                dm = a["heads"] * a["hd"]
                self.calls.append((lib.tfimm_hip_class_attention,
                                   (self.tptr(op.inputs[0]), self.tptr(op.inputs[1]), self.tptr(op.output), B,
                                    a["n_tokens"], a["heads"], a["hd"], dm, 2 * dm, dm)))
            elif k == "copy_rows":
                self.calls.append((lib.tfimm_hip_copy_rows,
                                   (self.tptr(op.inputs[0]), self.tptr(op.output), B, a["src_rows"], a["dst_rows"],
                                    a["dst_row0"], a["d"])))
            elif k == "stem_pool":
                d = ffi.StemDesc()
                d.x, d.out = self.tptr(op.inputs[0]), self.tptr(op.output)
                d.wt, d.bias = self.cptr(op.consts["wt"]), self.cptr(op.consts["bias"])
                d.batch, d.Hp, d.Wp2, d.OH, d.OW, d.ldw = B, a["Hp"], a["Wp2"], a["OH"], a["OW"], a["ldw"]
                cast = next((o.attrs for o in prog.ops if o.kind == "cast_input" and o.output == op.inputs[0]), None)
                if cast is not None and cast["c_in"] == 3 and self.prog.input_shape[2] == 3:
                    ih, iw, _ = self.prog.input_shape
                    self._stem_raw = (d, d.x, ih, iw, cast["pad"][0], cast["pad"][2])
                self._keepalive.append(d)
                self.calls.append((lib.tfimm_hip_stem_conv_pool, (C.byref(d),)))
            elif k == "maxpool":
                self.calls.append((lib.tfimm_hip_maxpool,
                                   (self.tptr(op.inputs[0]), self.tptr(op.output), B, a["H"], a["W"], a["C"],
                                    a["k"], a["stride"], a["pad"], a["OH"], a["OW"])))
            elif k == "mean_rows":
                self.calls.append((lib.tfimm_hip_mean_rows,
                                   (self.tptr(op.inputs[0]), self.tptr(op.output), B, a["R"], a["C"], a["out_f32"])))
            elif k == "bcast_rows":
                self.calls.append((lib.tfimm_hip_bcast_rows,
                                   (self.cptr(op.consts["src"]), self.tptr(op.output), B, a["n_rows"], a["d"],
                                    a["dst_rows"])))
            elif k == "dwconv":
                sums_ptr = None
                if a["sums"] is not None:
                    sums_ptr = self.tptr(a["sums"])
                    self.calls.append(("memset", (sums_ptr, B * a["C"] * 8)))
                self.calls.append((lib.tfimm_hip_dwconv,
                                   (self.tptr(op.inputs[0]), self.cptr(op.consts["w"]), self.cptr(op.consts.get("bias")),
                                    self.tptr(op.output), sums_ptr, B, a["H"], a["W"], a["C"], a["k"], a["stride"],
                                    a["pad_t"], a["pad_l"], a["OH"], a["OW"], ffi.ACT[a["act"]])))
            elif k == "se_gate":
                self.calls.append((lib.tfimm_hip_se_gate,
                                   (self.tptr(op.inputs[0]), a["sums_fixed"], a["inv_count"], self.cptr(op.consts["w1"]),
                                    self.cptr(op.consts["b1"]), self.cptr(op.consts["w2"]), self.cptr(op.consts["b2"]),
                                    self.tptr(op.output), B, a["C"], a["rd"], ffi.ACT[a["act"]], ffi.ACT[a["gate_act"]])))
            elif k == "scale_channels":
                res = self.tptr(op.inputs[2]) if a["has_residual"] else None
                self.calls.append((lib.tfimm_hip_scale_channels,
                                   (self.tptr(op.inputs[0]), self.tptr(op.inputs[1]), res, self.tptr(op.output), B,
                                    a["R"], a["C"], a["act_after"])))
            elif k == "attention_probs":
                self.calls.append((lib.tfimm_hip_attention_probs,
                                   (self.tptr(op.inputs[0]), self.tptr(op.output), B, a["n_tokens"], a["heads"], a["hd"],
                                    a["scale"])))
            elif k == "group_norm":
                res = self.tptr(op.inputs[1]) if a["has_residual"] else None
                self.calls.append((lib.tfimm_hip_group_norm,
                                   (self.tptr(op.inputs[0]), self.cptr(op.consts["gamma"]), self.cptr(op.consts["beta"]),
                                    res, self.tptr(op.output), self.tptr(a["ws"]), B, a["rows"], a["C"], a["groups"],
                                    a["eps"], ffi.ACT[a["act"]], ffi.ACT[a["act_after"]])))
            elif k == "blur_pool":
                self.calls.append((lib.tfimm_hip_blur_pool,
                                   (self.tptr(op.inputs[0]), self.tptr(op.output), B, a["H"], a["W"], a["C"], a["stride"])))
            elif k == "avg_pool":
                self.calls.append((lib.tfimm_hip_avg_pool,
                                   (self.tptr(op.inputs[0]), self.tptr(op.output), B, a["H"], a["W"], a["C"], a["k"],
                                    a["stride"])))
            elif k == "eca_gate":
                self.calls.append((lib.tfimm_hip_eca_gate,
                                   (self.tptr(op.inputs[0]), 1.0, self.cptr(op.consts["w"]), self.tptr(op.output), B,
                                    a["C"], a["k"], ffi.ACT[a["gate_act"]])))
            elif k == "patch_merge_ln":
                self.calls.append((lib.tfimm_hip_patch_merge_ln,
                                   (self.tptr(op.inputs[0]), self.tptr(op.output), self.cptr(op.consts["gamma"]),
                                    self.cptr(op.consts["beta"]), B, a["H"], a["W"], a["C"], a["eps"])))
            elif k == "topk":
                pr = self.tptr(op.extra_outputs[1]) if a["probs"] else None
                self.calls.append((lib.tfimm_hip_topk,
                                   (self.tptr(op.inputs[0]), a["ld"], B * a["rows"], a["N"], a["k"], self.tptr(op.output),
                                    self.tptr(op.extra_outputs[0]), pr)))
            elif k == "l2_normalize":
                self.calls.append((lib.tfimm_hip_l2_normalize,
                                   (self.tptr(op.inputs[0]), a["E"], B * a["rows"], a["E"], self.tptr(op.output), a["E"])))
            elif k == "lora_delta":
                d = ffi.LoraDesc()
                x_t, out_t = prog.tensors[op.inputs[0]], prog.tensors[op.output]
                d.x, d.a, d.b = self.tptr(x_t.id), self.cptr(op.consts["a"]), self.cptr(op.consts["b"])
                d.out = self.tptr(out_t.id)
                d.M, d.K, d.N, d.Rp = B * a["rows"], a["K"], a["N"], a["Rp"]
                d.lda, d.lda_a, d.ldc = x_t.C, a["K"], out_t.C
                if a["has_residual"]:
                    d.residual, d.ldr = self.tptr(op.inputs[1]), prog.tensors[op.inputs[1]].C
                self._keepalive.append(d)
                self.calls.append((lib.tfimm_hip_lora_delta, (C.byref(d),)))
# ... 368 lines not shown
            d.mean_host, d.std_host = host
            d.B, d.Hs, d.Ws, d.c_in, d.H, d.W, d.c_out = B, Hs, Ws, c_in, H, W, self._input_patch[4]
            if self.prog.precision != "fp32":
                d.pad_t, d.pad_b, d.pad_l, d.pad_r = self._input_pad
            entry = self._resize_tabs[key] = (d, tabs, host)
        d = entry[0]
        d.in_ = x_dev.data_ptr()
        fn = "tfimm_hip_ref_preprocess_resize" if self.prog.precision == "fp32" else "tfimm_hip_preprocess_resize"
        return getattr(ffi.lib, fn + ("_aa" if aa else ""))(C.byref(d), st)

    def stage_mixed(self, images, norm) -> bool:
        from ..models.factory import resize_geometry
        ffi = self.ffi
        _, _, (method, crop_pct, *aa) = norm
        aa = bool(aa and aa[0])
        H, W, _ = self.prog.input_shape
        c_in = self._input_patch[3]
        if len(images) != self.batch or any(im.ndim != 3 or im.shape[2] != c_in or im.dtype != np.uint8 for im in images):
            raise ValueError(f"mixed resize input of {len(images)} images for a plan of batch {self.batch}, {c_in} channels")
        fp32 = self.prog.precision == "fp32"
        pad = (0, 0, 0, 0) if fp32 else tuple(self._input_pad)
        sizes = [im.shape[:2] for im in images]
        tabs = ffi.resize_batch_tables(sizes, [resize_geometry(s, (H, W), crop_pct) for s in sizes], (H, W), method, aa,
                                       c_in=c_in, pad=pad)
        return self._stage_records(self._mixed, norm, tabs, images, pad, ffi.ResizeBatchRec,
                                   ffi.ResizeBatchAADesc if aa else ffi.ResizeBatchDesc)

    def stage_regions(self, frames, boxes, box_indices, norm) -> bool:
        from ..models.factory import resize_geometry
        ffi = self.ffi
        _, _, (method, crop_pct, *aa) = norm
        aa = bool(aa and aa[0])
        H, W, _ = self.prog.input_shape
        c_in = self._input_patch[3]
        if any(f.ndim != 3 or f.shape[2] != c_in or f.dtype != np.uint8 for f in frames):
            raise ValueError(f"region resize input: frames must be uint8 (Hf, Wf, {c_in})")
        boxes, box_indices = ffi.check_boxes([f.shape[:2] for f in frames], boxes, box_indices)
        if boxes.shape[0] != self.batch:
            raise ValueError(f"region resize input of {boxes.shape[0]} boxes for a plan of batch {self.batch}")
        used, local = np.unique(box_indices, return_inverse=True)
        used_frames = [frames[int(f)] for f in used]
        fp32 = self.prog.precision == "fp32"
        pad = (0, 0, 0, 0) if fp32 else tuple(self._input_pad)
        geo = [resize_geometry((int(b[2] - b[0]), int(b[3] - b[1])), (H, W), crop_pct) for b in boxes]
        tabs = ffi.resize_region_tables([f.shape[:2] for f in used_frames], boxes, local.astype(np.int32), geo, (H, W), method,
                                        aa, c_in=c_in, pad=pad)
        return self._stage_records(self._regions, norm, tabs, used_frames, pad, ffi.ResizeRegionRec,
                                   ffi.ResizeRegionAADesc if aa else ffi.ResizeRegionDesc)

    def _stage_records(self, store, norm, tabs, sources, pad, rec_cls, desc_cls) -> bool:
        import torch
        ffi = self.ffi
        mean, std, (method, _, *aa) = norm
        aa = bool(aa and aa[0])
        H, W, _ = self.prog.input_shape
        c_in = self._input_patch[3]
        st = store.get(norm)
        grew = False
        if st is None:
            d = desc_cls()
            host = ((C.c_float * c_in)(*[float(v) for v in mean]), (C.c_float * c_in)(*[float(v) for v in std]))
            d.mean_host, d.std_host = host
            d.out = self._input_patch[1]
            d.B, d.c_in, d.H, d.W, d.c_out = self.batch, c_in, H, W, self._input_patch[4]
            d.pad_t, d.pad_b, d.pad_l, d.pad_r = pad
            if not aa:
                d.taps = 4 if method == "bicubic" else 2
            st = store[norm] = {"desc": d, "host": host, "aa": aa, "arena_cap": 0, "w_cap": 0, "taps_cap": 0, "lds_cap": 0}
            grew = True
        d = st["desc"]
        arena_cap = _grown(tabs["in_bytes"], st["arena_cap"], 1 << 16)
        w_cap = _grown(tabs["w"].size, st["w_cap"], 1 << 14)
        if arena_cap != st["arena_cap"]:
            st["arena"] = torch.empty(arena_cap, dtype=torch.uint8, device=self.device)
            st["stage"] = torch.empty(arena_cap, dtype=torch.uint8, pin_memory=self.device != "cpu")
            st["arena_cap"], grew = arena_cap, True
            d.in_, d.in_bytes = st["arena"].data_ptr(), arena_cap
        n_rec = self.batch * C.sizeof(rec_cls)
        n_tab = tabs["idx"].size if not aa else tabs["start"].size
        if w_cap != st["w_cap"]:
            n_meta = n_rec + 4 * n_tab * (2 if aa else 1) + 4 * w_cap
            st["meta"] = torch.empty(n_meta, dtype=torch.uint8, device=self.device)
            st["meta_stage"] = torch.empty(n_meta, dtype=torch.uint8, pin_memory=self.device != "cpu")
            st["w_cap"], grew = w_cap, True
            base = st["meta"].data_ptr()
            d.recs = base
            if aa:
                d.start, d.count, d.w, d.w_floats = base + n_rec, base + n_rec + 4 * n_tab, base + n_rec + 8 * n_tab, w_cap
            else:
                d.idx, d.w = base + n_rec, base + n_rec + 4 * n_tab
        if aa:
            taps_cap = min(_grown(tabs["max_taps"], st["taps_cap"], 16), ffi.RESIZE_AA_MAX_TAPS)
            lds_cap = min(_grown(4 * tabs["lds_floats"], st["lds_cap"], 16 << 10), 64 << 10)
            if (taps_cap, lds_cap) != (st["taps_cap"], st["lds_cap"]):
                st["taps_cap"], st["lds_cap"], grew = taps_cap, lds_cap, True
                d.taps_cap, d.lds_bytes = taps_cap, lds_cap
        stage, pos = st["stage"].numpy(), 0
        for im in sources:
            stage[pos:pos + im.size] = im.reshape(-1)
            pos += im.size
        assert pos == tabs["in_bytes"]
        st["arena"][:pos].copy_(st["stage"][:pos], non_blocking=True)
        parts = [tabs["recs"]] + ([tabs["start"], tabs["count"]] if aa else [tabs["idx"]]) + [tabs["w"]]
        meta, pos = st["meta_stage"].numpy(), 0
        for a in parts:
            meta[pos:pos + a.nbytes] = a.view(np.uint8).reshape(-1)
            pos += a.nbytes
        st["meta"][:pos].copy_(st["meta_stage"][:pos], non_blocking=True)
        torch.cuda.current_stream().synchronize() if self.device != "cpu" else None
        return grew

    def _launch_mixed(self, st, norm) -> int:
        m = self._mixed.get(norm)
        if m is None:
            raise RuntimeError("run(MIXED) before stage_mixed: the plan holds no mixed batch for this norm")
        fn = "tfimm_hip_ref_preprocess_resize_batch" if self.prog.precision == "fp32" else "tfimm_hip_preprocess_resize_batch"
        return getattr(self.ffi.lib, fn + ("_aa" if m["aa"] else ""))(C.byref(m["desc"]), st)

    def _launch_regions(self, st, norm) -> int:
        m = self._regions.get(norm)
        if m is None:
            raise RuntimeError("run(REGIONS) before stage_regions: the plan holds no boxes for this norm")
        fn = "tfimm_hip_ref_preprocess_regions" if self.prog.precision == "fp32" else "tfimm_hip_preprocess_regions"
        return getattr(self.ffi.lib, fn + ("_aa" if m["aa"] else ""))(C.byref(m["desc"]), st)

    def run(self, x_dev, stream_ptr: Optional[int] = None, norm=None, lo: int = 0, hi: Optional[int] = None):
        import torch
        ffi = self.ffi
        if stream_ptr is None:
            stream_ptr = torch.cuda.current_stream().cuda_stream
        st = C.c_void_p(stream_ptr)
        idx = self._input_patch[0]
        marks = self._roctx_labels() if os.environ.get("TFIMM_ROCTX", "0") == "1" else None
        hi = len(self.calls) if hi is None else hi
        for i in range(lo, hi):
            fn, args = self.calls[i]
            if marks is not None:
                ffi.roctx_push(marks[i])
            try:
                if i == idx:
                    rc = self.launch_input(x_dev, st, norm)
                elif fn == "memset":
                    ffi.check(_hip_memset_async(args[0], args[1], stream_ptr), "hipMemsetAsync")
                    continue
                else:
                    rc = fn(*args, st)
            finally:
                if marks is not None:
                    ffi.roctx_pop()
            if rc != 0:
                ffi.check(rc, f"op {i} ({getattr(fn, '__name__', fn)})")

    def _roctx_labels(self) -> List[str]:
        labels, ops = [], iter(self.prog.ops)
        for fn, _ in self.calls:
            if fn == "memset":
                labels.append("memset (squeeze sums)")
                continue
            op = next(ops)
            labels.append(f"{len(labels)} {op.kind} {op.cite}".strip())
        return labels


class CapturedPlan:

    def __init__(self, plan: "Plan", x_dev, norm=None, sink=None):
        import torch
        self.plan = plan
        self.static_input = x_dev
        plan.run(x_dev, norm=norm)
        torch.cuda.synchronize()
        self.graph = torch.cuda.CUDAGraph()
        with torch.cuda.graph(self.graph, capture_error_mode="thread_local"):
            plan.run(x_dev, norm=norm)
            _record_sink(sink, lambda t: plan.tensor_view(t))

    def replay(self):
        self.graph.replay()


class CapturedBranches:

    def __init__(self, plans: List["Plan"], x_dev, norm=None, sink=None):
        import torch
        self.plans = plans
        self.static_input = x_dev
        bounds = np.cumsum([0] + [p.batch for p in plans])
        assert bounds[-1] == x_dev.shape[0], (bounds, tuple(x_dev.shape))
        self.slices = [(int(bounds[i]), int(bounds[i + 1])) for i in range(len(plans))]
        for p, (lo, hi) in zip(plans, self.slices):
            p.run(x_dev[lo:hi], norm=norm)
        torch.cuda.synchronize()
        self.side = [torch.cuda.Stream() for _ in plans[1:]]
        self.graph = torch.cuda.CUDAGraph()
        with torch.cuda.graph(self.graph, capture_error_mode="thread_local"):
            main = torch.cuda.current_stream()
            for s in self.side:
                s.wait_stream(main)
            lo, hi = self.slices[0]
            plans[0].run(x_dev[lo:hi], norm=norm)
            for s, p, (lo, hi) in zip(self.side, plans[1:], self.slices[1:]):
                with torch.cuda.stream(s):
                    p.run(x_dev[lo:hi], norm=norm)
            for s in self.side:
                main.wait_stream(s)
            if sink is not None:
                t, dst = sink
                for p, (lo, hi) in zip(plans, self.slices):
                    dst[lo:hi].copy_(p.tensor_view(t).view(dst[lo:hi].shape))

    def replay(self):
        self.graph.replay()

    def output(self, t: "TRef"):
        import torch
        return torch.cat([p.tensor_view(t) for p in self.plans], dim=0)


class CapturedHybrid:

    def __init__(self, prog: "Program", x_dev, cut_op: int, norm=None, sink=None):
        import torch
        B = x_dev.shape[0]
        assert 0 < cut_op <= len(prog.ops) and B >= 2
        self.full = Plan(prog, B)
        nb = branch_sizes(B, 2)
        live = prog.live_across(cut_op) if cut_op < len(prog.ops) else [t.id for t in prog.tensors if t.keep and t.dtype != "raw"]
        live = [t for t in live if prog.tensors[t].dtype != "raw"]
        self.halves, lo = [], 0
        for n_img in nb:
            ext = {t: self.full.tptr(t) + lo * prog.tensors[t].bytes_per_image for t in live}
            self.halves.append(Plan(prog, n_img, external=ext))
            lo += n_img
        self.static_input = x_dev
        self.cut_op = cut_op
        self.slices = [(0, nb[0]), (nb[0], B)]
        cut = self.full.op_call_start[cut_op] if cut_op < len(prog.ops) else len(self.full.calls)
        assert all(h.op_call_start == self.full.op_call_start for h in self.halves)
        self.cut_call = cut

        def forward():
            main = torch.cuda.current_stream()
            self.side.wait_stream(main)
            (a0, a1), (b0, b1) = self.slices
            self.halves[0].run(x_dev[a0:a1], norm=norm, hi=cut)
            with torch.cuda.stream(self.side):
                self.halves[1].run(x_dev[b0:b1], norm=norm, hi=cut)
            main.wait_stream(self.side)
            if cut < len(self.full.calls):
                self.full.run(x_dev, norm=norm, lo=cut)

        self.side = torch.cuda.Stream()
        self.full.run(x_dev, norm=norm)
        forward()
        torch.cuda.synchronize()
        self.graph = torch.cuda.CUDAGraph()
        with torch.cuda.graph(self.graph, capture_error_mode="thread_local"):
            forward()
            _record_sink(sink, lambda t: self.full.tensor_view(t))

    def replay(self):
        self.graph.replay()

    def output(self, t: "TRef"):
        return self.full.tensor_view(t)


def _record_sink(sink, view):
    if sink is not None:
        t, dst = sink
        dst.copy_(view(t).view(dst.shape))


def _hip_memset_async(ptr: int, nbytes: int, stream_ptr: int) -> int:
    from . import ffi
    return ffi.lib.tfimm_hip_memset_async(C.c_void_p(ptr), 0, nbytes, C.c_void_p(stream_ptr))
```

Before: 73980 images/sec.

## Fuse following 1x1 reduce conv into the C1=64 conv chain kernel

Extends the 3x3+1x1 chain kernel with a NEXT variant that also computes the next block's 1x1 256->64 reduce conv, reusing the epilogue output staged in LDS. The 256-channel activation no longer has to be re-read from memory by a separate gemm launch, and one launch per fused pair goes away. The cost is a longer pipeline schedule that interleaves w3 weight steps, more registers for the extra accumulator, and extra LDS writes in the epilogue. The planner detects eligible conv_chain+gemm pairs in ResNet stage 1 and allocates both outputs.

```diff
diff --git a/include/tfimm_hip.h b/include/tfimm_hip.h
--- a/include/tfimm_hip.h
+++ b/include/tfimm_hip.h
@@ -328,6 +328,16 @@
 } tfimm_chain_desc;
 
 TFIMM_API int tfimm_hip_conv_chain(const tfimm_chain_desc* d, void* stream);
+
+typedef struct tfimm_chain_next_desc {
+  tfimm_chain_desc chain;
+  const void* w3;
+  const float* b3;
+  void* out2;
+  int32_t N3, ldw3, ldc2;
+} tfimm_chain_next_desc;
+
+TFIMM_API int tfimm_hip_conv_chain_next(const tfimm_chain_next_desc* d, void* stream);
 
 typedef struct tfimm_expand_dw_desc {
   const void* x;
diff --git a/tensorflow-image-models_amd/csrc/gemm_chain.hip b/tensorflow-image-models_amd/csrc/gemm_chain.hip
--- a/tensorflow-image-models_amd/csrc/gemm_chain.hip
+++ b/tensorflow-image-models_amd/csrc/gemm_chain.hip
@@ -20,9 +20,15 @@
 
 int tfimm_launch_conv_strip_chain(const tfimm_chain_desc& d, int64_t M, int num_cu, hipStream_t stream);
 
-extern "C" int tfimm_hip_conv_chain(const tfimm_chain_desc* dp, void* stream) {
-  if (!dp) TFIMM_FAIL(TFIMM_EINVAL, "conv_chain: null descriptor");
-  const tfimm_chain_desc& d = *dp;
+namespace {
+struct ChainNext {
+  const void* w3;
+  const float* b3;
+  void* out2;
+  int N3, ldw3, ldc2;
+};
+
+int conv_chain_impl(const tfimm_chain_desc& d, const ChainNext* nx, void* stream) {
   if (!d.x || !d.w1 || !d.b1 || !d.w2 || !d.b2 || !d.out) TFIMM_FAIL(TFIMM_EINVAL, "conv_chain: null pointer");
   if (d.B <= 0 || d.H <= 0 || d.W <= 0 || d.Cin <= 0 || d.KH <= 0 || d.KW <= 0 || d.stride <= 0 || d.OH <= 0 || d.OW <= 0 ||
       d.C1 <= 0 || d.N2 <= 0)
@@ -33,6 +39,7 @@
     if (d.W > 31) TFIMM_FAIL(TFIMM_EUNSUP, "conv_chain: C1 = 128 needs W <= 31 (W = %d): the strip of a 128-pixel tile must fit 192 LDS rows", d.W);
     if (d.N2 != 256 && d.N2 != 512) TFIMM_FAIL(TFIMM_EUNSUP, "conv_chain: N2 = %d (built: 256, 512)", d.N2);
     if (d.ds_x || d.ds_w) TFIMM_FAIL(TFIMM_EUNSUP, "conv_chain: the shortcut-convolution flavour exists for C1 = 64 only");
+    if (nx) TFIMM_FAIL(TFIMM_EUNSUP, "conv_chain_next: the following 1x1 convolution is built into the C1 = 64 kernel only");
     if (d.ldw1 != 1152) TFIMM_FAIL(TFIMM_EINVAL, "conv_chain: ldw1 = %d, expected KH*KW*Cin = 1152", d.ldw1);
     if (d.ldw2 < 128 || (d.ldw2 & 7)) TFIMM_FAIL(TFIMM_EINVAL, "conv_chain: ldw2 = %d", d.ldw2);
     if (d.ldc < d.N2 || (d.ldc & 7) || (d.residual && (d.ldr < d.N2 || (d.ldr & 7))))
@@ -52,7 +59,7 @@
         c.x = (const char*)d.x + b0 * d.H * d.W * 256;
         c.out = (char*)d.out + b0 * d.OH * d.OW * d.ldc * 2;
         if (d.residual) c.residual = (const char*)d.residual + b0 * d.OH * d.OW * d.ldr * 2;
-        const int rc = tfimm_hip_conv_chain(&c, stream);
+        const int rc = conv_chain_impl(c, nullptr, stream);
         if (rc != 0) return rc;
       }
       return 0;
@@ -85,10 +92,23 @@
     TFIMM_FAIL(TFIMM_EUNSUP, "conv_chain: the shortcut-convolution flavour is built with relu activations");
   if (w1_bytes > 0x7fffff00LL || w2_bytes > 0x7fffff00LL)
     TFIMM_FAIL(TFIMM_EUNSUP, "conv_chain: a weight tensor exceeds the 2 GiB a buffer descriptor addresses");
+  int64_t w3_bytes = 0, out2_bytes = 0;
+  if (nx) {
+    if (!nx->w3 || !nx->b3 || !nx->out2) TFIMM_FAIL(TFIMM_EINVAL, "conv_chain_next: null pointer");
+    if (ds) TFIMM_FAIL(TFIMM_EUNSUP, "conv_chain_next: not built for the shortcut-convolution flavour");
+    if (!(d.act1 == TFIMM_ACT_RELU && d.act2 == TFIMM_ACT_RELU)) TFIMM_FAIL(TFIMM_EUNSUP, "conv_chain_next: built with relu activations");
+    if (d.N2 != 256 || nx->N3 != 64) TFIMM_FAIL(TFIMM_EUNSUP, "conv_chain_next: N2 = %d, N3 = %d (built: 256 -> 64)", d.N2, nx->N3);
+    if (nx->ldw3 < d.N2 || (nx->ldw3 & 7) || nx->ldc2 < nx->N3 || (nx->ldc2 & 7))
+      TFIMM_FAIL(TFIMM_EINVAL, "conv_chain_next: ldw3 = %d, ldc2 = %d", nx->ldw3, nx->ldc2);
+    if (((uintptr_t)nx->w3 | (uintptr_t)nx->b3 | (uintptr_t)nx->out2) & 15) TFIMM_FAIL(TFIMM_EINVAL, "conv_chain_next: pointers must be 16-byte aligned");
+    w3_bytes = (int64_t)nx->N3 * nx->ldw3 * 2;
+    out2_bytes = ((M - 1) * nx->ldc2 + nx->N3) * 2;
+  }
   static const int64_t limit = getenv("TFIMM_CHAIN_LIMIT") ? std::min<int64_t>(atoll(getenv("TFIMM_CHAIN_LIMIT")), 0x7fffff00LL) : 0x7fffff00LL;
-  if (M > limit || x_bytes > limit || out_bytes > limit || res_bytes > limit) {
+  if (M > limit || x_bytes > limit || out_bytes > limit || res_bytes > limit || out2_bytes > limit) {
     const int64_t per_img = std::max<int64_t>(std::max<int64_t>((int64_t)d.H * d.W * d.Cin * 2, (int64_t)d.OH * d.OW * d.ldc * 2),
-                                              d.residual ? (int64_t)d.OH * d.OW * d.ldr * 2 : 0);
+                                              std::max<int64_t>(d.residual ? (int64_t)d.OH * d.OW * d.ldr * 2 : 0,
+                                                                nx ? (int64_t)d.OH * d.OW * nx->ldc2 * 2 : 0));
     const int64_t chunk = limit / per_img;
     if (chunk < 1 || d.B <= 1) TFIMM_FAIL(TFIMM_EUNSUP, "conv_chain: one image exceeds the 2 GiB a buffer descriptor addresses");
     for (int64_t b0 = 0; b0 < d.B; b0 += chunk) {
@@ -98,7 +118,9 @@
       c.out = (char*)d.out + b0 * d.OH * d.OW * d.ldc * 2;
       if (d.residual) c.residual = (const char*)d.residual + b0 * d.OH * d.OW * d.ldr * 2;
       if (d.ds_x) c.ds_x = (const char*)d.ds_x + b0 * d.OH * d.OW * d.ds_cin * 2;
-      const int rc = tfimm_hip_conv_chain(&c, stream);
+      ChainNext cn;
+      if (nx) { cn = *nx; cn.out2 = (char*)nx->out2 + b0 * d.OH * d.OW * nx->ldc2 * 2; }
+      const int rc = conv_chain_impl(c, nx ? &cn : nullptr, stream);
       if (rc != 0) return rc;
     }
     return 0;
@@ -107,6 +129,8 @@
   ChainArgs a;
   a.x = (const bf16_t*)d.x; a.w1 = (const bf16_t*)d.w1; a.b1 = d.b1;
   a.w2 = (const bf16_t*)d.w2; a.b2 = d.b2; a.residual = (const bf16_t*)d.residual; a.out = (bf16_t*)d.out;
+  a.w3 = nx ? (const bf16_t*)nx->w3 : nullptr; a.b3 = nx ? nx->b3 : nullptr; a.out2 = nx ? (bf16_t*)nx->out2 : nullptr;
+  a.ldw3 = nx ? nx->ldw3 : 0; a.ldc2 = nx ? nx->ldc2 : 0; a.w3_bytes = (unsigned)w3_bytes; a.out2_bytes = (unsigned)out2_bytes;
   a.ds_x = (const bf16_t*)d.ds_x; a.ds_w = (const uint4*)d.ds_w; a.ds_bytes = ds ? (unsigned)(M * 128) : 0u;
   a.M = (int)M; a.N2 = d.N2;
   a.B = d.B; a.H = d.H; a.W = d.W;
@@ -122,12 +146,13 @@
 
   const int vi = d.N2 == 512;
   const int ri = (d.act1 == TFIMM_ACT_RELU && d.act2 == TFIMM_ACT_RELU) ? 1 : 0;
-  const gemm_chain_fn fn = ds ? (vi ? gemm_chain_kernel<8, TFIMM_ACT_RELU, true> : gemm_chain_kernel<4, TFIMM_ACT_RELU, true>)
+  const gemm_chain_fn fn = nx ? gemm_chain_kernel<4, TFIMM_ACT_RELU, false, true>
+                           : ds ? (vi ? gemm_chain_kernel<8, TFIMM_ACT_RELU, true> : gemm_chain_kernel<4, TFIMM_ACT_RELU, true>)
                            : ri ? (vi ? gemm_chain_kernel<8, TFIMM_ACT_RELU> : gemm_chain_kernel<4, TFIMM_ACT_RELU>)
                                 : (vi ? gemm_chain_kernel<8> : gemm_chain_kernel<4>);
   const int lds = ChainGeom::LDS_BYTES;
-  static tfimm_once_t ready[2][3];
-  const int fi = ds ? 2 : ri;
+  static tfimm_once_t ready[2][4];
+  const int fi = nx ? 3 : ds ? 2 : ri;
   if (ready[vi][fi].need()) {
     TFIMM_HIP_CHECK(hipFuncSetAttribute((const void*)fn, hipFuncAttributeMaxDynamicSharedMemorySize, lds));
     ready[vi][fi].mark();
@@ -138,3 +163,15 @@
   TFIMM_LAUNCH(fn, dim3((unsigned)grid), dim3(256), (size_t)lds, (hipStream_t)stream, a);
   return 0;
 }
+}
+
+extern "C" int tfimm_hip_conv_chain(const tfimm_chain_desc* dp, void* stream) {
+  if (!dp) TFIMM_FAIL(TFIMM_EINVAL, "conv_chain: null descriptor");
+  return conv_chain_impl(*dp, nullptr, stream);
+}
+
+extern "C" int tfimm_hip_conv_chain_next(const tfimm_chain_next_desc* dp, void* stream) {
+  if (!dp) TFIMM_FAIL(TFIMM_EINVAL, "conv_chain_next: null descriptor");
+  const ChainNext nx = {dp->w3, dp->b3, dp->out2, dp->N3, dp->ldw3, dp->ldc2};
+  return conv_chain_impl(dp->chain, &nx, stream);
+}
diff --git a/tensorflow-image-models_amd/csrc/gemm_chain_kernel.h b/tensorflow-image-models_amd/csrc/gemm_chain_kernel.h
--- a/tensorflow-image-models_amd/csrc/gemm_chain_kernel.h
+++ b/tensorflow-image-models_amd/csrc/gemm_chain_kernel.h
@@ -13,6 +13,11 @@
   const bf16_t* ds_x;
   const uint4* ds_w;
   bf16_t* out;
+  const bf16_t* w3;
+  const float* b3;
+  bf16_t* out2;
+  int ldw3, ldc2;
+  unsigned w3_bytes, out2_bytes;
   int M, N2;
   int B, H, W;
   int ldw1, ldw2, ldr, ldc;
@@ -52,9 +57,11 @@
   static constexpr int value = I;
 };
 
-template <int NS2, int ACT = -1, bool DS = false>
+template <int NS2, int ACT = -1, bool DS = false, bool NEXT = false>
 __global__ void __launch_bounds__(256, 2) gemm_chain_kernel(const ChainArgs p) {
   using G = ChainGeom;
+  static_assert(!NEXT || (!DS && ACT == TFIMM_ACT_RELU && G::WTN == 64), "NEXT: plain flavour, relu compiled in, one 64-column pass");
+  constexpr int NXT = NEXT ? 1 : 0;
   constexpr int BM = G::BM, NW = G::NW, STAGE = G::STAGE, BN2 = G::BN2, NST = G::NST;
   constexpr int TN1 = 2;
   constexpr int STRIP_INSTR = G::STRIP_ROWS / 8 / NW;
@@ -91,8 +98,11 @@
   const __amdgpu_buffer_rsrc_t rsrc_w2 = make_rsrc(p.w2, p.w2_bytes);
   const __amdgpu_buffer_rsrc_t rsrc_o = make_rsrc(p.out, p.out_bytes);
   const __amdgpu_buffer_rsrc_t rsrc_r = DS ? make_rsrc(p.ds_x, p.ds_bytes) : make_rsrc(p.residual, p.res_bytes);
+  const __amdgpu_buffer_rsrc_t rsrc_w3 = NEXT ? make_rsrc(p.w3, p.w3_bytes) : rsrc_w2;
+  const __amdgpu_buffer_rsrc_t rsrc_o2 = NEXT ? make_rsrc(p.out2, p.out2_bytes) : rsrc_o;
 
   static_assert(NS2 >= 2, "the counted waits below are derived for at least two GEMM-2 steps");
+  constexpr int T = NK1 + NS2 * (1 + NXT);
   constexpr int LOOK = NST - 1;
   const int lrow = lane >> 3, lpc = lane & 7;
 
@@ -107,6 +117,12 @@
   for (int j = 0; j < B2_INSTR; ++j) {
     const int r = (wave * B2_INSTR + j) * 8 + lrow;
     b2_off[j] = (unsigned)(((size_t)r * p.ldw2 + (lpc ^ ((r >> 1) & 7)) * 8) * 2);
+  }
+  unsigned b3_off[B2_INSTR];
+#pragma unroll
+  for (int j = 0; j < B2_INSTR; ++j) {
+    const int r = (wave * B2_INSTR + j) * 8 + lrow;
+    b3_off[j] = NEXT ? (unsigned)(((size_t)r * p.ldw3 + (lpc ^ ((r >> 1) & 7)) * 8) * 2) : 0u;
   }
 #pragma unroll
   for (int j = 0; j < STRIP_INSTR; ++j) {
@@ -129,8 +145,8 @@
   int iss_stage = 0;
   auto issue_step = [&](auto sc, int tile) __attribute__((always_inline)) {
     constexpr int S = decltype(sc)::value;
-    constexpr int SL = S >= NK1 + NS2 ? S - NK1 - NS2 : S;
-    const bool valid = S >= NK1 + NS2 ? (tile + t_step < t_hi) : true;
+    constexpr int SL = S >= T ? S - T : S;
+    const bool valid = S >= T ? (tile + t_step < t_hi) : true;
     char* const sa = sRing + iss_stage * STAGE;
     if constexpr (SL < NK1) {
 #pragma unroll
@@ -138,8 +154,13 @@
         const unsigned off = valid ? b1_off[j] : kOobOffset;
         __builtin_amdgcn_raw_ptr_buffer_load_lds(rsrc_w1, (lds_ptr_t)(sa + (wave * B1_INSTR + j) * 1024), 16, (int)off, SL * 128, 0, 0);
       }
+    } else if constexpr (NEXT && ((SL - NK1) & 1)) {
+#pragma unroll
+      for (int j = 0; j < B2_INSTR; ++j)
+        __builtin_amdgcn_raw_ptr_buffer_load_lds(rsrc_w3, (lds_ptr_t)(sa + (wave * B2_INSTR + j) * 1024), 16, (int)b3_off[j],
+                                                 ((SL - NK1) / 2) * 128, 0, 0);
     } else {
-      const int soff = (int)((size_t)(SL - NK1) * BN2 * p.ldw2 * 2);
+      const int soff = (int)((size_t)((SL - NK1) / (1 + NXT)) * BN2 * p.ldw2 * 2);
 #pragma unroll
       for (int j = 0; j < B2_INSTR; ++j)
         __builtin_amdgcn_raw_ptr_buffer_load_lds(rsrc_w2, (lds_ptr_t)(sa + (wave * B2_INSTR + j) * 1024), 16, (int)b2_off[j], soff, 0, 0);
@@ -160,27 +181,39 @@
   const bool has_res = !DS && p.residual != nullptr;
   float* const sEw = sEpi + wave * (G::EPI_WAVE / 4);
 
+  constexpr int STORES3 = NEXT ? ITS : 0, B3_LOADS = NEXT ? 2 : 0;
+  constexpr bool B1_TILE = DS || NEXT;
   struct Ops {
     static constexpr int all(int r) {
-      if (DS && r == NK1 - 2) return B1_INSTR + TN1 * 4;
+      if (B1_TILE && r == NK1 - 2) return B1_INSTR + TN1 * 4;
       if (r < NK1 - 1) return B1_INSTR;
       if (r == NK1 - 1) return EPI_LOADS + DS_X + B1_INSTR;
-      const int u = r - NK1;
+      const int u = (r - NK1) / (1 + NXT);
+      if (NEXT && ((r - NK1) & 1)) return u == NS2 - 1 ? B3_LOADS + B2_INSTR + STORES3 : B2_INSTR;
       return (u < NS2 - 1 ? EPI_LOADS : 0) + DS_W + B2_INSTR + (u == 0 ? STRIP_INSTR : 0) + STORES;
     }
     static constexpr int behind_dma(int r) {
       if (r < NK1) return 0;
-      return (r - NK1 == 0 ? STRIP_INSTR : 0) + STORES;
+      const int u = (r - NK1) / (1 + NXT);
+      if (NEXT && ((r - NK1) & 1)) return u == NS2 - 1 ? STORES3 : 0;
+      return (u == 0 ? STRIP_INSTR : 0) + STORES;
     }
     static constexpr int wait_for(int r) {
-      constexpr int T = NK1 + NS2;
       int n = behind_dma((r + T - LOOK) % T);
       for (int i = 1; i < LOOK; ++i) n += all((r + T - i) % T);
       return n;
     }
+    static constexpr int max_wait() {
+      int m = 0;
+      for (int r = 0; r < T; ++r) m = wait_for(r) > m ? wait_for(r) : m;
+      return m;
+    }
   };
   static_assert(B1_INSTR == B2_INSTR, "every weight step is two pieces per wave");
-  static_assert(Ops::wait_for(NK1 + NS2 - 1) < 64, "vmcnt is a 6-bit counter");
+  static_assert(Ops::max_wait() < 64, "vmcnt is a 6-bit counter");
+  static_assert(!NEXT || LOOK != 1 || (Ops::wait_for(0) == STORES3 && Ops::wait_for(NK1) == 0 && Ops::wait_for(NK1 + 1) == STRIP_INSTR + STORES &&
+                                       Ops::wait_for(NK1 + 2) == 0 && Ops::wait_for(NK1 + 3) == STORES && Ops::wait_for(T - 1) == STORES),
+                "NEXT: counted waits");
 
   f32x4 bias1[TN1][4];
   auto load_bias1 = [&]() __attribute__((always_inline)) {
@@ -192,7 +225,7 @@
         bias1[j][q] = f32x4{b4.x, b4.y, b4.z, b4.w};
       }
   };
-  if constexpr (!DS) {
+  if constexpr (!B1_TILE) {
     load_bias1();
     asm volatile("s_waitcnt vmcnt(0)" : "+v"(bias1[0][0]), "+v"(bias1[0][3]), "+v"(bias1[TN1 - 1][0]), "+v"(bias1[TN1 - 1][3])::"memory");
   }
@@ -260,7 +293,7 @@
       if constexpr (k < LOOK) { if (first) chain_wait_vm<(LOOK - 1) * B1_INSTR>(); else chain_wait_vm<Ops::wait_for(k)>(); }
       else chain_wait_vm<Ops::wait_for(k)>();
       tfimm_lds_reuse_barrier();
-      if constexpr (DS && k == NK1 - 2) { load_bias1(); __builtin_amdgcn_sched_barrier(0); }
+      if constexpr (B1_TILE && k == NK1 - 2) { load_bias1(); __builtin_amdgcn_sched_barrier(0); }
       if constexpr (k == NK1 - 1) {
         load_epi(ChainIdx<0>{});
         if constexpr (DS) {
@@ -318,11 +351,19 @@
         bmid[j * 2 + q2] = __builtin_bit_cast(bf16x8, pack8p(v));
       }
 
+    f32x16 acc3[TN2];
     auto slice_step = [&](auto uc) __attribute__((always_inline)) {
       constexpr int u = decltype(uc)::value;
       constexpr int n0 = u * BN2;
+      constexpr int R = NK1 + u * (1 + NXT);
       const unsigned out_off0 = (unsigned)(((size_t)em * p.ldc + n0 + e_c8 * 8) * 2);
-      chain_wait_vm<Ops::wait_for(NK1 + u)>();
+      if constexpr (NEXT && u == 0) {
+#pragma unroll
+        for (int j = 0; j < TN2; ++j)
+#pragma unroll
+          for (int e = 0; e < 16; ++e) acc3[j][e] = 0.f;
+      }
+      chain_wait_vm<Ops::wait_for(R)>();
       tfimm_lds_reuse_barrier();
       if constexpr (u + 1 < NS2) load_epi(ChainIdx<u + 1>{});
       u32x4 wds[TN2][4];
@@ -333,7 +374,7 @@
           for (int t = 0; t < 4; ++t) wds[j][t] = __builtin_bit_cast(u32x4, p.ds_w[(size_t)((u * TN2 + j) * 4 + t) * 64 + lane]);
       }
       __builtin_amdgcn_sched_barrier(0);
-      issue_step(ChainIdx<NK1 + u + LOOK>{}, tile);
+      issue_step(ChainIdx<R + LOOK>{}, tile);
       if constexpr (u == 0) issue_strip(tile + t_step, tile + t_step < t_hi);
       __builtin_amdgcn_sched_barrier(0);
 
@@ -411,17 +452,106 @@
           }
           act8p(v, act2p);
           const unsigned off = out_off0 + (unsigned)(it * RPI) * ldc2 + (unsigned)(g * WTN * 2);
-          __builtin_amdgcn_raw_buffer_store_b128(__builtin_bit_cast(u32x4, pack8p(v)), rsrc_o,
-                                                 (int)(skip_epi ? kOobOffset : off), 0, 0);
-        }
+          const u32x4 pk = __builtin_bit_cast(u32x4, pack8p(v));
+          __builtin_amdgcn_raw_buffer_store_b128(pk, rsrc_o, (int)(skip_epi ? kOobOffset : off), 0, 0);
+          if constexpr (NEXT) {
+            const int pr = it * RPI + e_row;
+            const unsigned addr = (unsigned)(size_t)(lds_ptr_t)(reinterpret_cast<char*>(sEw) + lds_slot(pr, e_c8) * 16);
+            asm volatile("ds_write_b128 %0, %1" ::"v"(addr), "v"(pk) : "memory");
+          }
+        }
+        }
+      }
+    };
+    auto next_step = [&](auto uc) __attribute__((always_inline)) {
+      constexpr int u = decltype(uc)::value;
+      constexpr int R = NK1 + 2 * u + 1;
+      constexpr bool last = u == NS2 - 1;
+      chain_wait_vm<Ops::wait_for(R)>();
+      tfimm_lds_reuse_barrier();
+      float4 b3raw[2];
+      if constexpr (last) {
+        b3raw[0] = *reinterpret_cast<const float4*>(p.b3 + e_c8 * 8);
+        b3raw[1] = *reinterpret_cast<const float4*>(p.b3 + e_c8 * 8 + 4);
+      }
+      __builtin_amdgcn_sched_barrier(0);
+      issue_step(ChainIdx<R + LOOK>{}, tile);
+      __builtin_amdgcn_sched_barrier(0);
+      u32x4 ub[KS2];
+      {
+        unsigned ra[KS2];
+#pragma unroll
+        for (int t = 0; t < KS2; ++t) ra[t] = (unsigned)(size_t)(lds_ptr_t)(reinterpret_cast<char*>(sEw) + lds_slot(frow, t * 2 + fhi) * 16);
+        asm volatile("ds_read_b128 %0, %4\n\tds_read_b128 %1, %5\n\tds_read_b128 %2, %6\n\tds_read_b128 %3, %7\n\t"
+                     "s_waitcnt lgkmcnt(0)"
+                     : "=&v"(ub[0]), "=&v"(ub[1]), "=&v"(ub[2]), "=&v"(ub[3])
+                     : "v"(ra[0]), "v"(ra[1]), "v"(ra[2]), "v"(ra[3]) : "memory");
+      }
+      {
+        const uint4* sW = reinterpret_cast<const uint4*>(sRing + cur * STAGE);
+#pragma unroll
+        for (int t = 0; t < KS2; ++t) {
+          bf16x8 fw[TN2];
+#pragma unroll
+          for (int j = 0; j < TN2; ++j) fw[j] = __builtin_bit_cast(bf16x8, sW[lds_slot(j * 32 + frow, t * 2 + fhi)]);
+#pragma unroll
+          for (int j = 0; j < TN2; ++j)
+            acc3[j] = __builtin_amdgcn_mfma_f32_32x32x16_bf16(fw[j], __builtin_bit_cast(bf16x8, ub[t]), acc3[j], 0, 0, 0);
+        }
+      }
+      rotate();
+      if constexpr (last) {
+        const unsigned out2_off0 = (unsigned)(((size_t)em * p.ldc2 + e_c8 * 8) * 2);
+        const unsigned ldc22 = (unsigned)p.ldc2 * 2u;
+        asm volatile("s_nop 15\n\ts_nop 3" : "+v"(acc3[0]), "+v"(acc3[TN2 - 1]));
+#pragma unroll
+        for (int j = 0; j < TN2; ++j)
+#pragma unroll
+          for (int q = 0; q < 4; ++q) {
+            const int slot = j * 8 + q * 2 + fhi;
+            const f32x4 v = {acc3[j][q * 4 + 0], acc3[j][q * 4 + 1], acc3[j][q * 4 + 2], acc3[j][q * 4 + 3]};
+            const unsigned addr = (unsigned)(size_t)(lds_ptr_t)(&sEw[frow * WTN + epi_slot(frow, slot) * 4]);
+            asm volatile("ds_write_b128 %0, %1" ::"v"(addr), "v"(v) : "memory");
+          }
+        const tfimm_f32x2 bias3[4] = {{b3raw[0].x, b3raw[0].y}, {b3raw[0].z, b3raw[0].w}, {b3raw[1].x, b3raw[1].y}, {b3raw[1].z, b3raw[1].w}};
+#pragma unroll
+        for (int ip = 0; ip < ITS; ip += 2) {
+          f32x4 st[4];
+          {
+            unsigned ra[4];
+#pragma unroll
+            for (int w = 0; w < 2; ++w) {
+              const int pr = (ip + w) * RPI + e_row;
+              ra[2 * w] = (unsigned)(size_t)(lds_ptr_t)(&sEw[pr * WTN + epi_slot(pr, 2 * e_c8) * 4]);
+              ra[2 * w + 1] = (unsigned)(size_t)(lds_ptr_t)(&sEw[pr * WTN + epi_slot(pr, 2 * e_c8 + 1) * 4]);
+            }
+            asm volatile("ds_read_b128 %0, %4\n\tds_read_b128 %1, %5\n\tds_read_b128 %2, %6\n\tds_read_b128 %3, %7\n\t"
+                         "s_waitcnt lgkmcnt(0)"
+                         : "=&v"(st[0]), "=&v"(st[1]), "=&v"(st[2]), "=&v"(st[3])
+                         : "v"(ra[0]), "v"(ra[1]), "v"(ra[2]), "v"(ra[3]) : "memory");
+          }
+#pragma unroll
+          for (int w = 0; w < 2; ++w) {
+            const int it = ip + w;
+            const f32x4 lo = st[2 * w], hi = st[2 * w + 1];
+            tfimm_f32x2 v[4] = {{lo[0], lo[1]}, {lo[2], lo[3]}, {hi[0], hi[1]}, {hi[2], hi[3]}};
+#pragma unroll
+            for (int e = 0; e < 4; ++e) v[e] += bias3[e];
+            act8p(v, act2p);
+            __builtin_amdgcn_raw_buffer_store_b128(__builtin_bit_cast(u32x4, pack8p(v)), rsrc_o2,
+                                                   (int)(out2_off0 + (unsigned)(it * RPI) * ldc22), 0, 0);
+          }
         }
       }
     };
     slice_step(ChainIdx<0>{});
+    if constexpr (NEXT) next_step(ChainIdx<0>{});
     slice_step(ChainIdx<1>{});
-    if constexpr (NS2 > 2) slice_step(ChainIdx<2>{});
-    if constexpr (NS2 > 3) slice_step(ChainIdx<3>{});
+    if constexpr (NEXT) next_step(ChainIdx<1>{});
+    if constexpr (NS2 > 2) { slice_step(ChainIdx<2>{}); if constexpr (NEXT) next_step(ChainIdx<2>{}); }
+    if constexpr (NS2 > 3) { slice_step(ChainIdx<3>{}); if constexpr (NEXT) next_step(ChainIdx<3>{}); }
     if constexpr (NS2 > 4) { slice_step(ChainIdx<4>{}); slice_step(ChainIdx<5>{}); slice_step(ChainIdx<6>{}); slice_step(ChainIdx<7>{}); }
+    static_assert(!NEXT || NS2 <= 4, "NEXT is instantiated for N2 = 256");
     static_assert(NS2 == 2 || NS2 == 3 || NS2 == 4 || NS2 == 8, "instantiate the slice steps of this NS2");
     first = false;
   }
diff --git a/tensorflow-image-models_amd/csrc/plan.hip b/tensorflow-image-models_amd/csrc/plan.hip
--- a/tensorflow-image-models_amd/csrc/plan.hip
+++ b/tensorflow-image-models_amd/csrc/plan.hip
@@ -70,6 +70,7 @@
   static const std::map<std::string, Entry> t = {
       TFIMM_ADAPTER_DESC(tfimm_hip_gemm, tfimm_gemm_desc),
       TFIMM_ADAPTER_DESC(tfimm_hip_conv_chain, tfimm_chain_desc),
+      TFIMM_ADAPTER_DESC(tfimm_hip_conv_chain_next, tfimm_chain_next_desc),
       TFIMM_ADAPTER_DESC(tfimm_hip_mlp_fused, tfimm_mlp_desc),
       TFIMM_ADAPTER_DESC(tfimm_hip_gemm_mx, tfimm_gemm_mx_desc),
       TFIMM_ADAPTER_DESC(tfimm_hip_expand_dwconv, tfimm_expand_dw_desc),
diff --git a/tensorflow-image-models_amd/tfimm/engine/ffi.py b/tensorflow-image-models_amd/tfimm/engine/ffi.py
--- a/tensorflow-image-models_amd/tfimm/engine/ffi.py
+++ b/tensorflow-image-models_amd/tfimm/engine/ffi.py
@@ -76,6 +76,13 @@
     ]
 
 
+class ChainNextDesc(C.Structure):
+    _fields_ = ChainDesc._fields_ + [
+        ("w3", C.c_void_p), ("b3", C.c_void_p), ("out2", C.c_void_p),
+        ("N3", C.c_int32), ("ldw3", C.c_int32), ("ldc2", C.c_int32),
+    ]
+
+
 class ExpandDwDesc(C.Structure):
     _fields_ = [
         ("x", C.c_void_p), ("w1", C.c_void_p), ("b1", C.c_void_p), ("wdw", C.c_void_p), ("b2", C.c_void_p),
@@ -191,6 +198,7 @@
     "tfimm_hip_device_info": (_i, [_i, C.c_char_p, _i]),
     "tfimm_hip_gemm": (_i, [C.POINTER(GemmDesc), _vp]),
     "tfimm_hip_conv_chain": (_i, [C.POINTER(ChainDesc), _vp]),
+    "tfimm_hip_conv_chain_next": (_i, [C.POINTER(ChainNextDesc), _vp]),
     "tfimm_hip_mlp_fused": (_i, [C.POINTER(MlpDesc), _vp]),
     "tfimm_hip_gemm_mx": (_i, [C.POINTER(GemmMxDesc), _vp]),
     "tfimm_hip_quantize_mx": (_i, [_vp, _i64, _i, _i64, _vp, _vp, _f, _vp, _vp, _i, _vp]),
diff --git a/tensorflow-image-models_amd/tfimm/engine/graph.py b/tensorflow-image-models_amd/tfimm/engine/graph.py
--- a/tensorflow-image-models_amd/tfimm/engine/graph.py
+++ b/tensorflow-image-models_amd/tfimm/engine/graph.py
@@ -111,7 +111,26 @@
     def weight_bytes(self) -> int:
         return sum(c.nbytes for c in self.consts)
 
-    def plan_buffers(self) -> Tuple[Dict[int, int], List[int]]:
+    def chain_next_pairs(self, split_at: Optional[int] = None) -> List[int]:
+        if self.precision == "fp32" or os.environ.get("TFIMM_NO_CHAIN_NEXT", "0") == "1":
+            return []
+        pairs = []
+        for i in range(len(self.ops) - 1):
+            c, g = self.ops[i], self.ops[i + 1]
+            ca, ga = c.attrs, g.attrs
+            if (c.kind != "conv_chain" or g.kind != "gemm" or i + 1 == split_at or c.extra_outputs
+                    or (ca["C1"], ca["N2"], ca["act1"], ca["act2"]) != (64, 256, "relu", "relu") or ca.get("has_ds")):
+                continue
+            if (g.inputs != [c.output] or ga.get("mode") != 0 or (ga["K"], ga["N"], ga["ldw"], ga["lda"]) != (256, 64, 256, 256)
+                    or ga["act"] != "relu" or ga["out_f32"] or "bias" not in g.consts or set(g.consts) - {"wt", "bias"}
+                    or any(ga.get(k) for k in ("has_residual", "has_scale", "remap", "dual", "res_mod", "ln", "a_byte_offset", "out_col",
+                                                 "out_byte_offset", "ldc"))
+                    or ga["M"] != ca["OH"] * ca["OW"] or self.tensors[g.output].C != 64):
+                continue
+            pairs.append(i)
+        return pairs
+
+    def plan_buffers(self, fused=()) -> Tuple[Dict[int, int], List[int]]:
         last_use: Dict[int, int] = {}
         for i, op in enumerate(self.ops):
             for t in op.inputs:
@@ -123,6 +142,8 @@
         assign: Dict[int, int] = {}
         for i, op in enumerate(self.ops):
             outs = ([op.output] if op.output is not None else []) + op.extra_outputs
+            if i in fused:
+                outs = outs + [self.ops[i + 1].output]
             for out in outs:
                 if out in assign:
                     continue
@@ -1025,7 +1046,8 @@
 
 
 class Plan:
-    def __init__(self, prog: Program, batch: int, device: str = "cuda", external: Optional[Dict[int, int]] = None):
+    def __init__(self, prog: Program, batch: int, device: str = "cuda", external: Optional[Dict[int, int]] = None,
+                 split_at: Optional[int] = None):
         import torch
         from . import ffi
         self.ffi = ffi
@@ -1035,7 +1057,8 @@
         self.batch = batch
         self.device = device
         prog.upload(device)
-        assign, slabs = prog.plan_buffers()
+        self.fused_next = frozenset(prog.chain_next_pairs(split_at))
+        assign, slabs = prog.plan_buffers(self.fused_next)
         self.slab_bytes = [s * batch for s in slabs]
         self.slabs = [torch.empty(max(n, 16), dtype=torch.uint8, device=device) for n in self.slab_bytes]
         self.assign = assign
@@ -1084,10 +1107,12 @@
     def _build(self):
         ffi, lib, B = self.ffi, self.ffi.lib, self.batch
         prog = self.prog
-        for op in prog.ops:
+        for oi, op in enumerate(prog.ops):
             a = op.attrs
             k = op.kind
             self.op_call_start.append(len(self.calls))
+            if oi - 1 in self.fused_next:
+                continue
             if k == "cast_input":
                 out = self.tptr(op.output)
                 H, W, cin = prog.input_shape
@@ -1185,7 +1210,8 @@
                 self._keepalive.append(d)
                 self.calls.append((lib.tfimm_hip_gemm_mx, (C.byref(d),)))
             elif k == "conv_chain":
-                d = ffi.ChainDesc()
+                nxt = prog.ops[oi + 1] if oi in self.fused_next else None
+                d = ffi.ChainNextDesc() if nxt is not None else ffi.ChainDesc()
                 d.x = self.tptr(op.inputs[0])
                 d.w1, d.b1 = self.cptr(op.consts["w1"]), self.cptr(op.consts["b1"])
                 d.w2, d.b2 = self.cptr(op.consts["w2"]), self.cptr(op.consts["b2"])
@@ -1198,7 +1224,12 @@
                 d.C1, d.N2, d.ldw1, d.ldw2, d.ldr, d.ldc = a["C1"], a["N2"], a["ldw1"], a["ldw2"], a["N2"], a["N2"]
                 d.act1, d.act2 = ffi.ACT[a["act1"]], ffi.ACT[a["act2"]]
                 self._keepalive.append(d)
-                self.calls.append((lib.tfimm_hip_conv_chain, (C.byref(d),)))
+                if nxt is not None:
+                    d.w3, d.b3, d.out2 = self.cptr(nxt.consts["wt"]), self.cptr(nxt.consts["bias"]), self.tptr(nxt.output)
+                    d.N3, d.ldw3, d.ldc2 = nxt.attrs["N"], nxt.attrs["ldw"], prog.tensors[nxt.output].C
+                    self.calls.append((lib.tfimm_hip_conv_chain_next, (C.byref(d),)))
+                else:
+                    self.calls.append((lib.tfimm_hip_conv_chain, (C.byref(d),)))
             elif k == "mlp_fused":
                 d = ffi.MlpDesc()
                 d.x, d.residual, d.out = self.tptr(op.inputs[0]), self.tptr(op.inputs[1]), self.tptr(op.output)
@@ -1873,13 +1904,17 @@
                 ffi.check(rc, f"op {i} ({getattr(fn, '__name__', fn)})")
 
     def _roctx_labels(self) -> List[str]:
-        labels, ops = [], iter(self.prog.ops)
+        labels, ops = [], iter(enumerate(self.prog.ops))
         for fn, _ in self.calls:
             if fn == "memset":
                 labels.append("memset (squeeze sums)")
                 continue
-            op = next(ops)
-            labels.append(f"{len(labels)} {op.kind} {op.cite}".strip())
+            oi, op = next(ops)
+            label = f"{len(labels)} {op.kind} {op.cite}"
+            if oi in self.fused_next:
+                nxt = next(ops)[1]
+                label += f" + {nxt.kind} {nxt.cite}"
+            labels.append(label.strip())
         return labels
 
 
@@ -1944,14 +1979,14 @@
         import torch
         B = x_dev.shape[0]
         assert 0 < cut_op <= len(prog.ops) and B >= 2
-        self.full = Plan(prog, B)
+        self.full = Plan(prog, B, split_at=cut_op)
         nb = branch_sizes(B, 2)
         live = prog.live_across(cut_op) if cut_op < len(prog.ops) else [t.id for t in prog.tensors if t.keep and t.dtype != "raw"]
         live = [t for t in live if prog.tensors[t].dtype != "raw"]
         self.halves, lo = [], 0
         for n_img in nb:
             ext = {t: self.full.tptr(t) + lo * prog.tensors[t].bytes_per_image for t in live}
-            self.halves.append(Plan(prog, n_img, external=ext))
+            self.halves.append(Plan(prog, n_img, external=ext, split_at=cut_op))
             lo += n_img
         self.static_input = x_dev
         self.cut_op = cut_op
```

Result: faster. 76040 images/sec, median of 6 (+2.8%).
